# Yifei-Y/Openset-RCNN

Hardware: AMD Instinct MI355X
Metric: images/sec at 3x800x1333, R50-FPN, 1/2/4/8 MI355X; mAP_k vs ref (higher is better)
Workload: dtype f16; 1 GPU; VOC-COCO openset_rcnn_R50_FPN_128k.yaml, inference-only, 3x800x1333 uint8 BGR -> padded 800x1344, 1000 proposals/level (4273/img), 1000 dets/img, 50+50 final; batch_per_gpu=16, global_batch=16, parallelism=dp1 (images sharded, no collective), detections_last_step=1600, unknown_detections_last_step=800, known_detections_last_step=800, micro_batch_streams=1, hipgraph=True, ranks=1, distinct_gpus=1, passes_in_flight=4, images_in_flight=64

## Files before the change

include/osr.h:

```cpp
#ifndef OSR_H_
#define OSR_H_

#include <stdint.h>

#ifdef __cplusplus
extern "C" {
#endif

#define OSR_ABI_VERSION 1

typedef int32_t osr_status;
enum {
    OSR_OK = 0,
    OSR_ERR_INVALID_ARG = -1,
    OSR_ERR_UNSUPPORTED = -2,
    OSR_ERR_LAUNCH = -3,
    OSR_ERR_WORKSPACE = -4
};

typedef enum { OSR_F32 = 0, OSR_F16 = 1, OSR_BF16 = 2 } osr_dtype;

#define OSR_MAX_LEVELS 8

int32_t osr_abi_version(void);
const char* osr_last_error(void);

int32_t osr_stem_padded_width(int32_t wp);
osr_status osr_preprocess(const void* src, int32_t src_is_u8, int32_t n, int32_t h, int32_t w, int32_t hp, int32_t wp,
                          const float mean[3], const float std[3], void* dst, int32_t dst_dtype, void* stream);

typedef struct osr_conv_params {
    int32_t n, hi, wi, cin;
    int32_t ho, wo, cout;
    int32_t kh, kw, stride_h, stride_w, pad_h, pad_w;
    int64_t in_stride_n, in_stride_h, in_stride_w;
    int64_t out_stride_n, out_stride_h, out_stride_w;
    int64_t res_stride_n, res_stride_h, res_stride_w;
    int32_t relu;
    int32_t res_mode;
    int32_t pad_mode;
    int32_t in_dtype;
    int32_t out_dtype;
    int32_t concurrency;
    void* workspace;
    int64_t workspace_bytes;
    const int32_t* row_seg_counts;
    int32_t row_seg_rows;
} osr_conv_params;

int64_t osr_conv2d_fwd_workspace_bytes(const osr_conv_params* p);
int32_t osr_conv2d_fwd_describe(const osr_conv_params* p, int32_t has_workspace, char* buf, int32_t buf_bytes);

osr_status osr_conv2d_fwd(const osr_conv_params* p, const void* in, const void* weight, const float* bias,
                          const void* residual, void* out, void* stream);
osr_status osr_conv2d_fwd_masked(const osr_conv_params* p, const void* in, const void* weight, const float* bias,
                                 const void* residual, const void* mask, void* out, void* stream);

osr_status osr_conv2d_chain_fwd(const osr_conv_params* p, const void* in, const void* weight, const float* bias, const void* w3,
                                const float* bias3, int32_t cout3, const void* residual, void* out, void* stream);
osr_status osr_conv2d_chain_fwd_ex(const osr_conv_params* p, const void* in, const void* weight, const float* bias, const void* w3,
                                   const float* bias3, int32_t cout3, const void* residual, void* out, void* mid_out,
                                   void* stream);

typedef struct osr_bottleneck_params {
    int32_t n, h, w;
    int32_t cin, cmid, cout;
    int32_t dtype;
    int32_t has_proj;
} osr_bottleneck_params;
osr_status osr_bottleneck_fwd(const osr_bottleneck_params* p, const void* in, const void* w1, const float* b1,
                              const void* w2, const float* b2, const void* w3, const float* b3, const void* wsc,
                              const float* bsc, void* out, void* stream);

int64_t osr_resize_tmp_bytes(int32_t rows, int32_t nw);
osr_status osr_resize_bilinear_u8(const uint8_t* in, int32_t h, int32_t w, int64_t in_row_stride, const int32_t* xbounds,
                                  const int32_t* xcoef, int32_t kx, const int32_t* ybounds, const int32_t* ycoef,
                                  int32_t ky, int32_t y_first, int32_t y_rows, int32_t nh, int32_t nw, uint8_t* tmp,
                                  int64_t tmp_bytes, uint8_t* out, void* stream);

osr_status osr_resize_bilinear_u8_planar(const uint8_t* in, int32_t planes, int32_t h, int32_t w, const int32_t* xbounds,
                                         const int32_t* xcoef, int32_t kx, const int32_t* ybounds, const int32_t* ycoef,
                                         int32_t ky, int32_t y_first, int32_t y_rows, int32_t nh, int32_t nw, int32_t mirror,
                                         uint8_t* tmp, int64_t tmp_bytes, uint8_t* out, void* stream);

osr_status osr_stem_maxpool_fwd(const void* xpad, int32_t n, int32_t hp, int32_t wp, const void* w_view, int32_t w_rows, const float* bias,
                                void* out, int32_t dtype, void* stream);
osr_status osr_stem_maxpool_fwd_raw(const void* src, int32_t src_is_u8, int32_t n, int32_t h, int32_t w, int32_t hp, int32_t wp,
                                    const float mean[3], const float std[3], const void* w_view, int32_t w_rows, const float* bias,
                                    void* out, int32_t dtype, void* stream);
osr_status osr_stem_pool_bwd(const void* s, const void* dpool, int32_t n, int32_t hs, int32_t ws, int32_t c, void* ds, int32_t dtype,
                             void* stream);
int64_t osr_stem_wgrad_workspace_bytes(int32_t n, int32_t hp, int32_t wp);
osr_status osr_stem_wgrad(const void* xpad, const void* ds, int32_t n, int32_t hp, int32_t wp, float* dw, int32_t accumulate, void* workspace,
                          int64_t workspace_bytes, int32_t dtype, void* stream);
osr_status osr_maxpool3x3s2(const void* in, int32_t n, int32_t hi, int32_t wi, int32_t c, void* out, int32_t dtype,
                            void* stream);
osr_status osr_subsample2(const void* in, int32_t n, int32_t hi, int32_t wi, int32_t c, void* out, int32_t dtype,
                          void* stream);

osr_status osr_gemm_f32(const float* a, int64_t lda, const float* w, const float* bias, float* out, int64_t ldo,
                        int32_t m, int32_t n, int32_t k, int32_t relu, void* stream);
int64_t osr_gemm_f32_tn_workspace_bytes(int32_t m, int32_t n, int32_t k);
osr_status osr_gemm_f32_tn(const float* a, int64_t lda, const float* b, int64_t ldb, float* out, int64_t ldo, int32_t m,
                           int32_t n, int32_t k, void* workspace, int64_t workspace_bytes, void* stream);

typedef struct osr_linear_split_params {
    int32_t m, n, k;
    int32_t relu;
    int64_t ldx, ldo;
    const int32_t* row_seg_counts;
    int32_t row_seg_rows;
    int32_t reserved;
} osr_linear_split_params;
osr_status osr_split_rows_bf16(const float* w, int32_t rows, int32_t cols, void* hi, void* lo, void* stream);
osr_status osr_linear_split_fwd(const osr_linear_split_params* p, const float* x, const void* w_hi, const void* w_lo,
                                const float* bias, float* out, void* stream);

osr_status osr_split_rows_bf16_t(const float* w, int32_t rows, int32_t cols, void* hi, void* lo, void* stream);
osr_status osr_linear_split_dgrad(const float* dy, int64_t lddy, const void* wt_hi, const void* wt_lo, const float* mask,
                                  int64_t ldmask, float* dx, int64_t lddx, int32_t m, int32_t n, int32_t k,
                                  const int32_t* row_seg_counts, int32_t row_seg_rows, void* stream);
int64_t osr_linear_split_wgrad_workspace_bytes(int32_t m, int32_t n, int32_t k);
osr_status osr_linear_split_wgrad(const float* dy, int64_t lddy, const float* x, int64_t ldx, float* dw, int64_t lddw,
                                  int32_t m, int32_t n, int32_t k, const int32_t* row_seg_counts, int32_t row_seg_rows,
                                  void* workspace, int64_t workspace_bytes, void* stream);

osr_status osr_conv2d_split_fwd(const osr_conv_params* p, const float* in, const void* w_hi, const void* w_lo,
                                const float* bias, const float* residual, float* out, void* stream);

osr_status osr_cfrpn_head_tail(const void* t, int32_t t_dtype, int64_t rows, int32_t c, const float* w_delta,
                               const float* b_delta, const float* w_ctr, const float* b_ctr, float* deltas,
                               float* ctr, void* stream);

osr_status osr_cfrpn_head_fwd(const osr_conv_params* p, const void* in, const void* weight, const float* bias,
                              const float* w_tail, const float* b_tail, float* deltas, float* ctr, void* stream);
osr_status osr_conv2d_fwd_pair(const osr_conv_params* p, const void* in, const void* w_a, const float* bias_a, int32_t cout_a,
                               int32_t relu_a, void* out_a, const void* w_b, const float* bias_b, int32_t cout_b, int32_t relu_b,
                               void* out_b, void* stream);

typedef struct osr_conv_level {
    const void* in;
    void* out;
    float* deltas;
    float* ctr;
    const void* weight;
    const float* bias;
    int32_t n, hi, wi;
    int32_t reserved;
} osr_conv_level;
#define OSR_MAX_CONV_LEVELS 6
osr_status osr_conv2d_fwd_levels(const osr_conv_params* p, int32_t nlevels, const osr_conv_level* levels, const void* weight,
                                 const float* bias, void* stream);
osr_status osr_cfrpn_head_fwd_levels(const osr_conv_params* p, int32_t nlevels, const osr_conv_level* levels, const void* weight,
                                     const float* bias, const float* w_tail, const float* b_tail, void* stream);
osr_status osr_cfrpn_head_fwd_ex(const osr_conv_params* p, const void* in, const void* weight, const float* bias,
                                 const float* w_tail, const float* b_tail, float* deltas, float* ctr, void* hidden_out,
                                 void* stream);

typedef struct osr_rpn_levels {
    int32_t num_levels;
    int32_t num_anchors;
    int32_t h[OSR_MAX_LEVELS];
    int32_t w[OSR_MAX_LEVELS];
    int32_t stride[OSR_MAX_LEVELS];
    int64_t offset[OSR_MAX_LEVELS];
} osr_rpn_levels;

int32_t osr_rpn_select_capacity(const osr_rpn_levels* lv, int32_t pre_nms_topk);
int64_t osr_rpn_select_workspace_bytes(const osr_rpn_levels* lv, int32_t n, int32_t pre_nms_topk);
osr_status osr_rpn_select(const osr_rpn_levels* lv, const float* cell_anchors , const float* ctr,
                          const float* deltas, int32_t n, const int32_t* image_hw , int32_t pre_nms_topk,
                          float min_box_size, float* boxes, float* scores, int32_t* src_index, int32_t* batch_idx,
                          int32_t* counts, int32_t* status_flags, void* workspace, int64_t workspace_bytes,
                          void* stream);

osr_status osr_rpn_select_ex(const osr_rpn_levels* lv, const float* cell_anchors, const float* ctr, const float* deltas,
                             int32_t n, const int32_t* image_hw, int32_t pre_nms_topk, float min_box_size,
                             int32_t decode_mode, const float reg_weights[4], float* boxes, float* scores,
                             int32_t* src_index, int32_t* batch_idx, int32_t* level_out, int32_t* counts,
                             int32_t* status_flags, void* workspace, int64_t workspace_bytes, void* stream);

typedef struct osr_pyramid {
    int32_t num_levels;
    int32_t c;
    int32_t h[OSR_MAX_LEVELS];
    int32_t w[OSR_MAX_LEVELS];
    float scale[OSR_MAX_LEVELS];
    const void* data[OSR_MAX_LEVELS];
} osr_pyramid;

#define OSR_ROI_MAX_POOLED_FWD 14
osr_status osr_roi_align_fwd(const osr_pyramid* feats, int32_t feat_dtype, int32_t n, const float* boxes,
                             const int32_t* batch_idx, int64_t m, int32_t pooled, int32_t canonical_level,
                             int32_t canonical_size, int32_t min_level, void* out, int32_t out_dtype, void* stream);

osr_status osr_roi_align_fwd_ordered(const osr_pyramid* feats, int32_t feat_dtype, int32_t n, const float* boxes,
                                     const int32_t* batch_idx, int64_t m, int32_t pooled, int32_t canonical_level,
                                     int32_t canonical_size, int32_t min_level, const int32_t* order,
                                     const int32_t* order_nvalid, void* out, int32_t out_dtype, void* stream);
#define OSR_ROI_NO_PADDING_FILL 1
osr_status osr_roi_align_fwd_ordered_ex(const osr_pyramid* feats, int32_t feat_dtype, int32_t n, const float* boxes,
                                        const int32_t* batch_idx, int64_t m, int32_t pooled, int32_t canonical_level,
                                        int32_t canonical_size, int32_t min_level, const int32_t* order,
                                        const int32_t* order_nvalid, int32_t flags, void* out, int32_t out_dtype, void* stream);
#define OSR_ROI_MAX_SAMPLING_RATIO 64
typedef struct osr_roi_options {
    int32_t aligned;
    int32_t sampling_ratio;
} osr_roi_options;
osr_status osr_roi_align_fwd_ordered_opt(const osr_pyramid* feats, int32_t feat_dtype, int32_t n, const float* boxes,
                                         const int32_t* batch_idx, int64_t m, int32_t pooled, int32_t canonical_level,
                                         int32_t canonical_size, int32_t min_level, const int32_t* order,
                                         const int32_t* order_nvalid, int32_t flags, const osr_roi_options* options, void* out,
                                         int32_t out_dtype, void* stream);
int64_t osr_roi_locality_order_workspace_bytes(int32_t n, int64_t m);
osr_status osr_roi_locality_order(const osr_pyramid* feats, int32_t n, const float* boxes, const int32_t* batch_idx, int64_t m,
                                  int32_t canonical_level, int32_t canonical_size, int32_t min_level, int32_t* order,
                                  int32_t* nvalid, void* workspace, int64_t workspace_bytes, void* stream);

osr_status osr_box_predictor_tail(const float* x, int64_t m, int32_t k, const float* w, const float* b,
                                  const float* proposals, const float* ctr, const int32_t* batch_idx,
                                  const int32_t* image_hw, const float reg_weights[4], int32_t mean_type,
                                  float score_thresh, float* pred_deltas, float* pred_iou, float* boxes,
                                  float* score, int32_t* cand, void* stream);

int64_t osr_nms_topk_workspace_bytes(int32_t num_segments, int64_t seg_stride);
osr_status osr_nms_topk(const float* boxes, const float* scores, const int32_t* cls ,
                        const int32_t* cand , int32_t num_segments, int64_t seg_stride,
                        const int32_t* seg_len, float thr, int32_t topk, int32_t* keep, int32_t* keep_count,
                        void* workspace, int64_t workspace_bytes, void* stream);

osr_status osr_gather_rows(const float* src, int64_t seg_stride, int32_t row_elems, const int32_t* keep,
                           const int32_t* keep_count, int32_t num_segments, int32_t topk, float* dst, void* stream);

osr_status osr_l2_normalize_rows(const float* x, int32_t rows, int32_t d, float* out, void* stream);

osr_status osr_pln_tail(const float* emb, int64_t rows, int32_t d, const float* protos_normed, int32_t num_known,
                        int32_t reps, float unk_thr, int64_t unknown_id, const int64_t* class_map,
                        const int32_t* rows_valid, int32_t seg_rows, int64_t* pred_class, float* min_dist,
                        void* stream);
enum { OSR_PLN_DIST_COS = 0, OSR_PLN_DIST_L1 = 1, OSR_PLN_DIST_L2 = 2 };
osr_status osr_pln_tail_ex(const float* emb, int64_t rows, int32_t d, const float* protos_normed, int32_t num_known,
                           int32_t reps, int32_t distance_type, float unk_thr, int64_t unknown_id,
                           const int64_t* class_map, const int32_t* rows_valid, int32_t seg_rows, int64_t* pred_class,
                           float* min_dist, void* stream);

osr_status osr_softmax_candidates(const float* logits, int32_t num_known, const float* det_boxes,
                                  const float* det_scores, const int64_t* pred_class, const int32_t* det_count,
                                  int32_t n, int32_t seg_rows, int64_t unknown_id, float known_thresh,
                                  float unknown_thresh, float* k_boxes, float* k_scores, int32_t* k_cls, int32_t* k_det,
                                  int32_t* k_count, float* u_boxes, float* u_scores, int32_t* u_det, int32_t* u_count,
                                  void* stream);

osr_status osr_fastrcnn_candidates(const float* logits, const float* deltas, int32_t num_classes,
                                   int32_t num_bbox_reg_classes, const float* prop_boxes, const int32_t* prop_count,
                                   int32_t n, int32_t seg_rows, const int32_t* image_hw, const float reg_weights[4],
                                   float score_thresh, float* c_boxes, float* c_scores, int32_t* c_cls, int32_t* c_row,
                                   int32_t* c_count, void* stream);

osr_status osr_assemble_detections(const float* k_boxes, const float* k_scores, const int32_t* k_cls,
                                   const int32_t* k_keep, const int32_t* k_keep_count, int64_t k_stride, int32_t k_topk,
                                   const float* u_boxes, const float* u_scores, const int32_t* u_keep,
                                   const int32_t* u_keep_count, int64_t u_stride, int32_t u_topk, int32_t n,
                                   int64_t unknown_id, const int64_t* class_map, float* out_boxes, float* out_scores,
                                   int64_t* out_classes, int32_t* out_count, void* stream);

osr_status osr_detector_postprocess(const float* boxes, const float* scores, const int64_t* classes, const int32_t* count,
                                    int32_t n, int32_t cap, const float* scale_xy, const int32_t* out_hw, float* out_boxes,
                                    float* out_scores, int64_t* out_classes, int32_t* out_count, void* stream);

osr_status osr_mask_upsample_predict(const void* x, int32_t dtype, int64_t r, int32_t s, int32_t cin, int32_t cmid,
                                     const void* w_packed, const float* bias, const float* pred_w, const float* pred_b,
                                     int32_t num_rows, const int64_t* classes, const int32_t* rows_valid, int32_t seg_rows,
                                     float* probs, void* stream);
osr_status osr_mask_upsample_predict_ex(const void* x, int32_t dtype, int64_t r, int32_t s, int32_t cin, int32_t cmid,
                                        const void* w_packed, const float* bias, const float* pred_w, const float* pred_b,
                                        int32_t num_rows, const int64_t* classes, const int32_t* rows_valid, int32_t seg_rows,
                                        float* probs, float* logits, void* stream);
osr_status osr_paste_masks(const float* probs, const float* boxes, int64_t r, int32_t m, int32_t out_h, int32_t out_w,
                           float threshold, uint8_t* out, void* stream);

int64_t osr_mask_upsample_predict_bwd_workspace_bytes(int64_t r, int32_t s, int32_t cmid);
osr_status osr_mask_upsample_predict_bwd(const void* x, int32_t dtype, int64_t r, int32_t s, int32_t cin, int32_t cmid,
                                         const void* w_packed, const void* w_packed_t, const float* bias, const float* pred_w,
                                         int32_t num_rows, const int64_t* classes, const int32_t* rows_valid, int32_t seg_rows,
                                         const float* d_logits, void* dx, int32_t dx_dtype, void* g_out, float* d_pred_w, float* d_pred_b,
                                         float* d_deconv_b, void* workspace, int64_t workspace_bytes, void* stream);
osr_status osr_mask_targets(const uint8_t* gt_masks, int32_t n, int32_t gmax, int32_t hm, int32_t wm, const int32_t* image_hw,
                            const float* boxes, const int32_t* gt_idx, const int32_t* rows_valid, int32_t seg_rows,
                            int32_t m_side, uint8_t* targets, void* stream);
osr_status osr_mask_loss_fwd(const float* logits, const uint8_t* targets, int64_t rows, int32_t m_side, int32_t num_rows,
                             const int64_t* classes, const int32_t* rows_valid, int32_t seg_rows, float loss_weight, float* out6,
                             void* workspace, int64_t workspace_bytes, void* stream);
osr_status osr_mask_loss_bwd(const float* logits, const uint8_t* targets, int64_t rows, int32_t m_side, int32_t num_rows,
                             const int64_t* classes, const int32_t* rows_valid, int32_t seg_rows, float scale, float* d_logits,
                             void* workspace, int64_t workspace_bytes, void* stream);

osr_status osr_tta_boxes_to_original(const float* boxes, const float* scores, const int64_t* classes, const int32_t* counts,
                                     const int32_t* sizes, int32_t n, int32_t topk, int32_t ha, int32_t wa, int32_t flip,
                                     int32_t slot, int32_t cap, float* c_boxes, float* c_scores, int32_t* c_cls,
                                     int32_t* c_cand, void* stream);
osr_status osr_tta_boxes_to_augmented(const float* boxes, const int32_t* counts, const int32_t* sizes, int32_t n, int32_t topk,
                                      int32_t ha, int32_t wa, int32_t flip, float* out, void* stream);
osr_status osr_tta_reduce_masks(const float* maps, const int32_t* flip, int32_t num_aug, const int32_t* counts, int32_t n,
                                int32_t topk, int32_t m, float* out, void* stream);


osr_status osr_rpn_match_anchors(const osr_rpn_levels* levels, const float* cell_anchors, int32_t n,
                                 const float* gt_boxes, const int32_t* gt_count, int32_t gmax, float reg_lo,
                                 float reg_hi, float obj_lo, float obj_hi, int32_t* matched_idx, float* matched_iou,
                                 int8_t* labels_reg, int8_t* labels_obj, void* workspace, int64_t workspace_bytes,
                                 void* stream);

osr_status osr_subsample_labels(int8_t* labels, const float* keys, int32_t n, int64_t r, int32_t num_samples,
                                float positive_fraction, int32_t* num_pos_out, int32_t* num_neg_out, void* stream);

osr_status osr_rpn_anchor_targets(const osr_rpn_levels* levels, const float* cell_anchors, int32_t n,
                                  const float* gt_boxes, const int32_t* gt_count, int32_t gmax,
                                  const int32_t* matched_idx, const int8_t* labels_obj, float* matched_boxes,
                                  float* ctr_target, void* stream);

osr_status osr_rpn_losses_fwd(const osr_rpn_levels* levels, const float* cell_anchors, int32_t n,
                              const float* pred_deltas, const float* pred_ctr, const int8_t* labels_reg,
                              const int8_t* labels_obj, const float* matched_boxes, const float* ctr_target,
                              float loc_weight, float ctr_weight, int32_t batch_size_per_image, float* out6,
                              void* workspace, int64_t workspace_bytes, void* stream);
enum { OSR_BOX_LOSS_IOU = 0, OSR_BOX_LOSS_SMOOTH_L1 = 1, OSR_BOX_LOSS_GIOU = 2, OSR_BOX_LOSS_DIOU = 3, OSR_BOX_LOSS_CIOU = 4 };
typedef struct osr_loss_options {
    int32_t box_loss_type;
    float box_smooth_l1_beta;
    float aux_smooth_l1_beta;
} osr_loss_options;
osr_status osr_rpn_losses_fwd_ex(const osr_rpn_levels* levels, const float* cell_anchors, int32_t n,
                                 const float* pred_deltas, const float* pred_ctr, const int8_t* labels_reg,
                                 const int8_t* labels_obj, const float* matched_boxes, const float* ctr_target,
                                 float loc_weight, float ctr_weight, int32_t batch_size_per_image,
                                 const osr_loss_options* options, float* out6, void* workspace, int64_t workspace_bytes,
                                 void* stream);

int64_t osr_roi_match_sample_workspace_bytes(int32_t n, int64_t pcap, int32_t gmax);
osr_status osr_roi_match_and_sample(const float* prop_boxes, const float* prop_logits, const int32_t* prop_count,
                                    int64_t pcap, const float* gt_boxes, const int64_t* gt_classes,
                                    const int32_t* gt_count, int32_t gmax, int32_t n, const float* keys,
                                    int32_t num_classes, int32_t batch_size, float positive_fraction, float iou_thr,
                                    float* out_boxes, float* out_logits, int64_t* out_classes, float* out_ious,
                                    float* out_gt_boxes, int32_t* out_src, int32_t* out_batch_idx, int32_t* out_counts,
                                    void* workspace, int64_t workspace_bytes, void* stream);
osr_status osr_roi_match_and_sample_ex(const float* prop_boxes, const float* prop_logits, const int32_t* prop_count,
                                       int64_t pcap, const float* gt_boxes, const int64_t* gt_classes,
                                       const int32_t* gt_count, int32_t gmax, int32_t n, const float* keys,
                                       int32_t num_classes, int32_t batch_size, float positive_fraction, float iou_thr,
                                       float* out_boxes, float* out_logits, int64_t* out_classes, float* out_ious,
                                       float* out_gt_boxes, int32_t* out_src, int32_t* out_batch_idx, int32_t* out_counts,
                                       int32_t* out_gt_idx, void* workspace, int64_t workspace_bytes, void* stream);

osr_status osr_roi_box_losses_fwd(const float* pred_deltas, int32_t delta_stride, const float* pred_iou,
                                  int32_t iou_stride, int32_t iou_is_logit, const float* proposal_boxes,
                                  const float* gt_boxes, const int64_t* gt_classes, const float* gt_iou, int64_t m,
                                  int32_t num_classes, const float reg_weights[4], float box_weight, float iou_weight,
                                  float* out3, void* workspace, int64_t workspace_bytes, void* stream);
osr_status osr_roi_box_losses_fwd_ex(const float* pred_deltas, int32_t delta_stride, const float* pred_iou,
                                     int32_t iou_stride, int32_t iou_is_logit, const float* proposal_boxes,
                                     const float* gt_boxes, const int64_t* gt_classes, const float* gt_iou, int64_t m,
                                     int32_t num_classes, const float reg_weights[4], float box_weight, float iou_weight,
                                     const osr_loss_options* options, float* out3, void* workspace,
                                     int64_t workspace_bytes, void* stream);

osr_status osr_pln_loss_fwd(const float* emb, int64_t m, int32_t d, const float* protos_normed, int32_t num_known,
                            const int64_t* gt_classes, const float* ious, float iou_thr, float alpha, float beta,
                            float loss_weight, float* out1, void* workspace, int64_t workspace_bytes, void* stream);
osr_status osr_pln_loss_fwd_ex(const float* emb, int64_t m, int32_t d, const float* protos_normed, int32_t num_known,
                               int32_t reps, int32_t distance_type, const int64_t* gt_classes, const float* ious,
                               float iou_thr, float alpha, float beta, float loss_weight, float* out1, void* workspace,
                               int64_t workspace_bytes, void* stream);

// ... 173 lines not shown
```

openset-rcnn_amd/csrc/osr_bottleneck.hip:

```cpp
#include "osr_common.h"

typedef float f32x4 __attribute__((ext_vector_type(4)));
typedef f16_t bnf16x8 __attribute__((ext_vector_type(8)));
typedef bf16_t bnbf16x8 __attribute__((ext_vector_type(8)));
typedef unsigned bnu32x4 __attribute__((ext_vector_type(4)));
typedef __attribute__((address_space(3))) void bn_lds_void_t;

template <class T> struct BnFrag;
template <> struct BnFrag<f16_t> {
    typedef bnf16x8 type;
    static __device__ __forceinline__ f32x4 mfma(bnf16x8 a, bnf16x8 b, f32x4 c) { return __builtin_amdgcn_mfma_f32_16x16x32_f16(a, b, c, 0, 0, 0); }
};
template <> struct BnFrag<bf16_t> {
    typedef bnbf16x8 type;
    static __device__ __forceinline__ f32x4 mfma(bnbf16x8 a, bnbf16x8 b, f32x4 c) { return __builtin_amdgcn_mfma_f32_16x16x32_bf16(a, b, c, 0, 0, 0); }
};

struct BnArgs {
    const void* x;
    void* y;
    const void *w1, *w2, *w3, *wsc;
    const float *b1, *b2, *b3, *bsc;
    int n, h, w;
    int tiles_y, tiles_x;
    unsigned x_bytes, y_bytes, w1_bytes, w2_bytes, w3_bytes, wsc_bytes;
#ifdef BN_STAMPS
    unsigned long long* dbg;
#endif
};

#ifdef BN_STAMPS
static unsigned long long* g_bn_stamps = nullptr;
extern "C" void osr_debug_set_bn_stamps(unsigned long long* p) { g_bn_stamps = p; }
#define BN_STAMP(i) if (a.dbg && tid == 0) a.dbg[(long long)blockIdx.x * 8 + (i)] = __builtin_amdgcn_s_memrealtime()
#else
#define BN_STAMP(i)
#endif

#define BN_TH 8
#define BN_TW 16
#define BN_HW 18
#define BN_NHALO 180
#define BN_MID1 0
#define BN_MID2 24576
#define BN_WBUF 40960
#define BN_BIAS 73728
#define BN_LDS (73728 + 384 * 4)
#define BN_OOB 0x80000000u

__device__ __forceinline__ int bn_nmap(int rho) {
    const int T = rho >> 4, i = rho & 15;
    return 32 * (T >> 1) + 8 * (i >> 2) + 4 * (T & 1) + (i & 3);
}

template <class TI> __device__ __forceinline__ typename BnFrag<TI>::type bn_as_frag(bnu32x4 v) {
    union { bnu32x4 u; typename BnFrag<TI>::type f; } c;
    c.u = v;
    return c.f;
}

template <class TI, int CIN, int PROJ>
__global__ __launch_bounds__(256, 2) void bottleneck64_kernel(BnArgs a) {
    typedef typename BnFrag<TI>::type frag_t;
    constexpr int NK32 = CIN / 32, NKS = CIN / 64;
    static_assert(CIN == 64 || CIN == 256, "res2 blocks only");
    static_assert(PROJ ? CIN == 64 : CIN == 256, "identity shortcut needs cin == cout");
    extern __shared__ __attribute__((aligned(1024))) unsigned char lds[];

    const int tid = threadIdx.x, lane = tid & 63;
    const int wid = __builtin_amdgcn_readfirstlane(tid >> 6);
    const int l15 = lane & 15, g = lane >> 4;
    BN_STAMP(0);

    int t;
    {
        const int nwg = gridDim.x, b = blockIdx.x, q = nwg >> 3, r = nwg & 7, xcd = b & 7, idx = b >> 3;
        t = (xcd < r ? xcd * (q + 1) : r * (q + 1) + (xcd - r) * q) + idx;
    }
    const int tx = t % a.tiles_x, ty = (t / a.tiles_x) % a.tiles_y, img = t / (a.tiles_x * a.tiles_y);
    const int y0 = ty * BN_TH, x0 = tx * BN_TW;

    const __amdgpu_buffer_rsrc_t rs_x = __builtin_amdgcn_make_buffer_rsrc(const_cast<void*>(a.x), 0, a.x_bytes, 0x00020000);
    const __amdgpu_buffer_rsrc_t rs_y = __builtin_amdgcn_make_buffer_rsrc(a.y, 0, a.y_bytes, 0x00020000);
    const __amdgpu_buffer_rsrc_t rs_w1 = __builtin_amdgcn_make_buffer_rsrc(const_cast<void*>(a.w1), 0, a.w1_bytes, 0x00020000);
    const __amdgpu_buffer_rsrc_t rs_w2 = __builtin_amdgcn_make_buffer_rsrc(const_cast<void*>(a.w2), 0, a.w2_bytes, 0x00020000);
    const __amdgpu_buffer_rsrc_t rs_w3 = __builtin_amdgcn_make_buffer_rsrc(const_cast<void*>(a.w3), 0, a.w3_bytes, 0x00020000);

    {
        const int lrow = lane >> 3, slot = lane & 7;
#pragma unroll
        for (int ks = 0; ks < NKS; ++ks)
#pragma unroll
            for (int j = 0; j < 2; ++j) {
                const int piece = wid * 2 + j;
                const int rho = piece * 8 + lrow;
                const unsigned chunk = (unsigned)(slot ^ ((rho >> 1) & 7));
                const unsigned voff = (unsigned)((bn_nmap(rho) * CIN + ks * 64 + (int)chunk * 8) * 2);
                __builtin_amdgcn_raw_ptr_buffer_load_lds(rs_w1, (bn_lds_void_t*)(lds + BN_WBUF + ks * 8192 + piece * 1024), 16, voff, 0, 0, 0);
            }
        float* s_bias = reinterpret_cast<float*>(lds + BN_BIAS);
        for (int i = tid; i < 384; i += 256) {
            float v;
            if (i < 64) v = a.b1[i];
            else if (i < 128) v = a.b2[i - 64];
            else v = a.b3[i - 128] + (PROJ ? a.bsc[i - 128] : 0.f);
            s_bias[i] = v;
        }
    }

    unsigned xoff[3];
    bool hvalid[3];
#pragma unroll
    for (int i = 0; i < 3; ++i) {
        const int hr = wid * 48 + i * 16 + l15;
        const int hy = hr / BN_HW, hx = hr - hy * BN_HW;
        const int gy = y0 - 1 + hy, gx = x0 - 1 + hx;
        hvalid[i] = hr < BN_NHALO && (unsigned)gy < (unsigned)a.h && (unsigned)gx < (unsigned)a.w;
        xoff[i] = hvalid[i] ? (unsigned)((((long long)img * a.h + gy) * a.w + gx) * CIN * 2 + g * 16) : BN_OOB;
    }
    frag_t xf[3][NK32];
#pragma unroll
    for (int k = 0; k < NK32; ++k)
#pragma unroll
        for (int i = 0; i < 3; ++i) xf[i][k] = bn_as_frag<TI>(__builtin_amdgcn_raw_buffer_load_b128(rs_x, xoff[i] + k * 64, 0, 0));

    asm volatile("s_waitcnt vmcnt(0)" ::: "memory");
    __syncthreads();
    BN_STAMP(1);

#define BN_SW(row, chunk) ((row) * 128 + ((((chunk)) ^ (((row) >> 1) & 7)) << 4))
    {
        f32x4 acc[3][4];
#pragma unroll
        for (int i = 0; i < 3; ++i)
#pragma unroll
            for (int T = 0; T < 4; ++T) acc[i][T] = f32x4{0.f, 0.f, 0.f, 0.f};
#pragma unroll
        for (int k = 0; k < NK32; ++k) {
            frag_t wf[4];
#pragma unroll
            for (int T = 0; T < 4; ++T) {
                const int rho = T * 16 + l15;
                wf[T] = *reinterpret_cast<const frag_t*>(lds + BN_WBUF + (k >> 1) * 8192 + BN_SW(rho, (k & 1) * 4 + g));
            }
#pragma unroll
            for (int i = 0; i < 3; ++i)
#pragma unroll
                for (int T = 0; T < 4; ++T) acc[i][T] = BnFrag<TI>::mfma(wf[T], xf[i][k], acc[i][T]);
        }
        const float* s_b1 = reinterpret_cast<const float*>(lds + BN_BIAS);
#pragma unroll
        for (int i = 0; i < 3; ++i) {
            const int hr = wid * 48 + i * 16 + l15;
#pragma unroll
            for (int p = 0; p < 2; ++p) {
                const float4 ba = *reinterpret_cast<const float4*>(s_b1 + 32 * p + 8 * g), bb = *reinterpret_cast<const float4*>(s_b1 + 32 * p + 8 * g + 4);
                const float bias[8] = {ba.x, ba.y, ba.z, ba.w, bb.x, bb.y, bb.z, bb.w};
                frag_t o;
#pragma unroll
                for (int e = 0; e < 8; ++e) {
                    const float v = (e < 4 ? acc[i][2 * p][e] : acc[i][2 * p + 1][e - 4]) + bias[e];
                    o[e] = (TI)(hvalid[i] ? fmaxf(v, 0.f) : 0.f);
                }
                *reinterpret_cast<frag_t*>(lds + BN_MID1 + BN_SW(hr, 4 * p + g)) = o;
            }
        }
    }
    __syncthreads();
    BN_STAMP(2);

    frag_t w3f[4][2];
    frag_t wscf[PROJ ? 4 : 1][2];
#pragma unroll
    for (int T = 0; T < 4; ++T)
#pragma unroll
        for (int k = 0; k < 2; ++k) {
            const int n = wid * 64 + bn_nmap(T * 16 + l15);
            w3f[T][k] = bn_as_frag<TI>(__builtin_amdgcn_raw_buffer_load_b128(rs_w3, (unsigned)((n * 64 + k * 32 + g * 8) * 2), 0, 0));
            if constexpr (PROJ) {
                const __amdgpu_buffer_rsrc_t rs_wsc = __builtin_amdgcn_make_buffer_rsrc(const_cast<void*>(a.wsc), 0, a.wsc_bytes, 0x00020000);
                wscf[T][k] = bn_as_frag<TI>(__builtin_amdgcn_raw_buffer_load_b128(rs_wsc, (unsigned)((n * CIN + k * 32 + g * 8) * 2), 0, 0));
            }
        }

#define BN_STAGE_TAP(tap_)                                                                                                          \
    {                                                                                                                               \
        const int lrow_ = lane >> 3, slot_ = lane & 7;                                                                              \
        _Pragma("unroll") for (int j_ = 0; j_ < 2; ++j_) {                                                                          \
            const int piece_ = wid * 2 + j_;                                                                                        \
            const int rho_ = piece_ * 8 + lrow_;                                                                                    \
            const unsigned chunk_ = (unsigned)(slot_ ^ ((rho_ >> 1) & 7));                                                          \
            const unsigned voff_ = (unsigned)(((bn_nmap(rho_) * 9 + (tap_)) * 64 + (int)chunk_ * 8) * 2);                            \
            __builtin_amdgcn_raw_ptr_buffer_load_lds(rs_w2, (bn_lds_void_t*)(lds + BN_WBUF + ((tap_) & 3) * 8192 + piece_ * 1024), 16, voff_, 0, 0, 0); \
        }                                                                                                                           \
    }
    BN_STAGE_TAP(0);
    BN_STAGE_TAP(1);
    BN_STAGE_TAP(2);
    {
        f32x4 acc[2][4];
#pragma unroll
        for (int j = 0; j < 2; ++j)
#pragma unroll
            for (int T = 0; T < 4; ++T) acc[j][T] = f32x4{0.f, 0.f, 0.f, 0.f};
#pragma unroll
        for (int tap = 0; tap < 9; ++tap) {
            if (tap <= 6) asm volatile("s_waitcnt vmcnt(4) lgkmcnt(0)\n\ts_barrier" ::: "memory");
            else if (tap == 7) asm volatile("s_waitcnt vmcnt(2) lgkmcnt(0)\n\ts_barrier" ::: "memory");
            else asm volatile("s_waitcnt vmcnt(0) lgkmcnt(0)\n\ts_barrier" ::: "memory");
            if (tap + 3 < 9) BN_STAGE_TAP(tap + 3);
            const int ky = tap / 3, kx = tap - ky * 3;
            const unsigned char* wb = lds + BN_WBUF + (tap & 3) * 8192;
            frag_t wf[4][2];
#pragma unroll
            for (int T = 0; T < 4; ++T)
#pragma unroll
                for (int k = 0; k < 2; ++k) wf[T][k] = *reinterpret_cast<const frag_t*>(wb + BN_SW(T * 16 + l15, k * 4 + g));
#pragma unroll
            for (int j = 0; j < 2; ++j) {
                const int hr = (wid * 2 + j + ky) * BN_HW + kx + l15;
#pragma unroll
                for (int k = 0; k < 2; ++k) {
                    const frag_t af = *reinterpret_cast<const frag_t*>(lds + BN_MID1 + BN_SW(hr, k * 4 + g));
#pragma unroll
                    for (int T = 0; T < 4; ++T) acc[j][T] = BnFrag<TI>::mfma(wf[T][k], af, acc[j][T]);
                }
            }
        }
        const float* s_b2 = reinterpret_cast<const float*>(lds + BN_BIAS) + 64;
#pragma unroll
        for (int j = 0; j < 2; ++j) {
            const int row = (wid * 2 + j) * 16 + l15;
#pragma unroll
            for (int p = 0; p < 2; ++p) {
                const float4 ba = *reinterpret_cast<const float4*>(s_b2 + 32 * p + 8 * g), bb = *reinterpret_cast<const float4*>(s_b2 + 32 * p + 8 * g + 4);
                const float bias[8] = {ba.x, ba.y, ba.z, ba.w, bb.x, bb.y, bb.z, bb.w};
                frag_t o;
#pragma unroll
                for (int e = 0; e < 8; ++e) o[e] = (TI)fmaxf((e < 4 ? acc[j][2 * p][e] : acc[j][2 * p + 1][e - 4]) + bias[e], 0.f);
                *reinterpret_cast<frag_t*>(lds + BN_MID2 + BN_SW(row, 4 * p + g)) = o;
            }
        }
    }
    __syncthreads();
    BN_STAMP(3);

    const float* s_b3 = reinterpret_cast<const float*>(lds + BN_BIAS) + 128 + wid * 64;
    float bias3[2][8];
#pragma unroll
    for (int p = 0; p < 2; ++p) {
        const float4 ba = *reinterpret_cast<const float4*>(s_b3 + 32 * p + 8 * g), bb = *reinterpret_cast<const float4*>(s_b3 + 32 * p + 8 * g + 4);
        bias3[p][0] = ba.x; bias3[p][1] = ba.y; bias3[p][2] = ba.z; bias3[p][3] = ba.w;
        bias3[p][4] = bb.x; bias3[p][5] = bb.y; bias3[p][6] = bb.z; bias3[p][7] = bb.w;
    }
    frag_t aux[2][2][2];
    unsigned ooff[2][2];
#define BN_FETCH(buf, gi_)                                                                                                          \
    {                                                                                                                               \
        _Pragma("unroll") for (int j_ = 0; j_ < 2; ++j_) {                                                                          \
            const int gy_ = y0 + 2 * (gi_) + j_, gx_ = x0 + l15;                                                                    \
            const bool ok_ = gy_ < a.h && gx_ < a.w;                                                                                \
            const long long pix_ = ((long long)img * a.h + gy_) * a.w + gx_;                                                        \
            ooff[buf][j_] = ok_ ? (unsigned)(pix_ * 256 * 2) : BN_OOB;                                                              \
            _Pragma("unroll") for (int q_ = 0; q_ < 2; ++q_) {                                                                      \
                const unsigned off_ = !ok_ ? BN_OOB : PROJ ? (unsigned)(pix_ * CIN * 2 + (q_ * 32 + g * 8) * 2)                      \
                                                           : (unsigned)(pix_ * 256 * 2 + (wid * 64 + 32 * q_ + 8 * g) * 2);          \
                aux[buf][j_][q_] = bn_as_frag<TI>(__builtin_amdgcn_raw_buffer_load_b128(rs_x, off_, 0, 0));                          \
            }                                                                                                                       \
        }                                                                                                                           \
    }
    BN_FETCH(0, 0);
#pragma unroll
    for (int gi = 0; gi < 4; ++gi) {
        const int cur = gi & 1;
        if (gi + 1 < 4) { BN_FETCH((gi + 1) & 1, gi + 1); }
        f32x4 acc[2][4];
#pragma unroll
        for (int j = 0; j < 2; ++j)
#pragma unroll
            for (int T = 0; T < 4; ++T) acc[j][T] = f32x4{0.f, 0.f, 0.f, 0.f};
#pragma unroll
        for (int j = 0; j < 2; ++j) {
            const int row = (2 * gi + j) * 16 + l15;
#pragma unroll
            for (int k = 0; k < 2; ++k) {
                const frag_t af = *reinterpret_cast<const frag_t*>(lds + BN_MID2 + BN_SW(row, k * 4 + g));
#pragma unroll
                for (int T = 0; T < 4; ++T) acc[j][T] = BnFrag<TI>::mfma(w3f[T][k], af, acc[j][T]);
            }
            if constexpr (PROJ) {
#pragma unroll
                for (int k = 0; k < 2; ++k)
#pragma unroll
                    for (int T = 0; T < 4; ++T) acc[j][T] = BnFrag<TI>::mfma(wscf[T][k], aux[cur][j][k], acc[j][T]);
            }
        }
#pragma unroll
        for (int j = 0; j < 2; ++j)
#pragma unroll
            for (int p = 0; p < 2; ++p) {
                frag_t o;
#pragma unroll
                for (int e = 0; e < 8; ++e) {
                    float v = (e < 4 ? acc[j][2 * p][e] : acc[j][2 * p + 1][e - 4]) + bias3[p][e];
                    if constexpr (!PROJ) v += (float)aux[cur][j][p][e];
                    o[e] = (TI)fmaxf(v, 0.f);
                }
                union { frag_t f; bnu32x4 u; } cv;
                cv.f = o;
                __builtin_amdgcn_raw_buffer_store_b128(cv.u, rs_y, ooff[cur][j] == BN_OOB ? BN_OOB : ooff[cur][j] + (unsigned)((wid * 64 + 32 * p + 8 * g) * 2), 0, 0);
            }
    }
    BN_STAMP(4);
#ifdef BN_STAMPS
    asm volatile("s_waitcnt vmcnt(0)" ::: "memory");
    BN_STAMP(5);
#endif
}

template <class TI>
static osr_status bottleneck_launch(const osr_bottleneck_params* p, BnArgs& a, hipStream_t st) {
    const unsigned grid = (unsigned)(a.n * a.tiles_y * a.tiles_x);
    if (p->has_proj) {
        static osr_dev_mask m{0};
        osr_once_per_device(m, [] { (void)hipFuncSetAttribute(reinterpret_cast<const void*>(bottleneck64_kernel<TI, 64, 1>), hipFuncAttributeMaxDynamicSharedMemorySize, BN_LDS); });
        hipLaunchKernelGGL((bottleneck64_kernel<TI, 64, 1>), dim3(grid), dim3(256), BN_LDS, st, a);
    } else {
        static osr_dev_mask m{0};
        osr_once_per_device(m, [] { (void)hipFuncSetAttribute(reinterpret_cast<const void*>(bottleneck64_kernel<TI, 256, 0>), hipFuncAttributeMaxDynamicSharedMemorySize, BN_LDS); });
        hipLaunchKernelGGL((bottleneck64_kernel<TI, 256, 0>), dim3(grid), dim3(256), BN_LDS, st, a);
    }
    OSR_CHECK_LAUNCH("osr_bottleneck_fwd");
    return OSR_OK;
}

extern "C" osr_status osr_bottleneck_fwd(const osr_bottleneck_params* p, const void* in, const void* w1, const float* b1, const void* w2,
                                         const float* b2, const void* w3, const float* b3, const void* wsc, const float* bsc, void* out,
                                         void* stream) {
    OSR_REQUIRE(p && in && w1 && b1 && w2 && b2 && w3 && b3 && out, OSR_ERR_INVALID_ARG, "osr_bottleneck_fwd: null pointer");
    OSR_REQUIRE(p->n >= 1 && p->h >= 1 && p->w >= 1, OSR_ERR_INVALID_ARG, "osr_bottleneck_fwd: bad geometry");
    OSR_REQUIRE(p->dtype == OSR_F16 || p->dtype == OSR_BF16, OSR_ERR_UNSUPPORTED, "osr_bottleneck_fwd: dtype must be f16/bf16");
    OSR_REQUIRE(p->cmid == 64 && p->cout == 256 && ((p->has_proj && p->cin == 64) || (!p->has_proj && p->cin == 256)), OSR_ERR_UNSUPPORTED,
                "osr_bottleneck_fwd: only the res2 shapes are fused (cmid 64, cout 256; cin 64 with a projection or cin 256 without): run "
                "three osr_conv2d_fwd launches instead");
    OSR_REQUIRE(!p->has_proj || (wsc && bsc), OSR_ERR_INVALID_ARG, "osr_bottleneck_fwd: the projection shortcut needs its weight and bias");
    OSR_REQUIRE(in != out, OSR_ERR_INVALID_ARG, "osr_bottleneck_fwd: in-place is not supported (neighbouring tiles read the halo)");
    OSR_REQUIRE((((uintptr_t)in | (uintptr_t)out | (uintptr_t)w1 | (uintptr_t)w2 | (uintptr_t)w3 | (uintptr_t)wsc | (uintptr_t)b1 | (uintptr_t)b2 | (uintptr_t)b3) & 15) == 0,
                OSR_ERR_INVALID_ARG, "osr_bottleneck_fwd: pointers must be 16-byte aligned");
    const long long px = (long long)p->n * p->h * p->w;
    const long long xb = px * p->cin * 2, yb = px * p->cout * 2;
    OSR_REQUIRE(xb < (1ll << 31) - 4096 && yb < (1ll << 31) - 4096, OSR_ERR_UNSUPPORTED, "osr_bottleneck_fwd: tensor too large for 32-bit buffer offsets");
    BnArgs a;
    a.x = in; a.y = out; a.w1 = w1; a.w2 = w2; a.w3 = w3; a.wsc = wsc; a.b1 = b1; a.b2 = b2; a.b3 = b3; a.bsc = bsc;
    a.n = p->n; a.h = p->h; a.w = p->w;
    a.tiles_y = (p->h + BN_TH - 1) / BN_TH; a.tiles_x = (p->w + BN_TW - 1) / BN_TW;
#ifdef BN_STAMPS
    a.dbg = g_bn_stamps;
#endif
    a.x_bytes = (unsigned)xb; a.y_bytes = (unsigned)yb;
    a.w1_bytes = (unsigned)(64 * p->cin * 2); a.w2_bytes = 64 * 9 * 64 * 2; a.w3_bytes = 256 * 64 * 2; a.wsc_bytes = (unsigned)(256 * p->cin * 2);
    OSR_REQUIRE((long long)a.n * a.tiles_y * a.tiles_x < (1ll << 31), OSR_ERR_UNSUPPORTED, "osr_bottleneck_fwd: too many tiles");
    hipStream_t st = (hipStream_t)stream;
    return p->dtype == OSR_F16 ? bottleneck_launch<f16_t>(p, a, st) : bottleneck_launch<bf16_t>(p, a, st);
}
```

openset-rcnn_amd/host/_lib.py:

```python
from __future__ import annotations

import ctypes as C
import os

import torch

PKG_DIR = os.path.dirname(os.path.dirname(os.path.abspath(__file__)))
LIB_PATH = os.path.join(PKG_DIR, "libosr_hip.so")

OSR_MAX_LEVELS = 8
OSR_F32, OSR_F16, OSR_BF16 = 0, 1, 2
ABI_VERSION = 1


class OsrError(RuntimeError):
    pass


ERR_UNSUPPORTED = -2


class ConvParams(C.Structure):
    _fields_ = [
        ("n", C.c_int32), ("hi", C.c_int32), ("wi", C.c_int32), ("cin", C.c_int32),
        ("ho", C.c_int32), ("wo", C.c_int32), ("cout", C.c_int32),
        ("kh", C.c_int32), ("kw", C.c_int32), ("stride_h", C.c_int32), ("stride_w", C.c_int32),
        ("pad_h", C.c_int32), ("pad_w", C.c_int32),
        ("in_stride_n", C.c_int64), ("in_stride_h", C.c_int64), ("in_stride_w", C.c_int64),
        ("out_stride_n", C.c_int64), ("out_stride_h", C.c_int64), ("out_stride_w", C.c_int64),
        ("res_stride_n", C.c_int64), ("res_stride_h", C.c_int64), ("res_stride_w", C.c_int64),
        ("relu", C.c_int32), ("res_mode", C.c_int32), ("pad_mode", C.c_int32),
        ("in_dtype", C.c_int32), ("out_dtype", C.c_int32), ("concurrency", C.c_int32),
        ("workspace", C.c_void_p), ("workspace_bytes", C.c_int64),
        ("row_seg_counts", C.c_void_p), ("row_seg_rows", C.c_int32),
    ]


class ConvLevel(C.Structure):
    _fields_ = [("in_", C.c_void_p), ("out", C.c_void_p), ("deltas", C.c_void_p), ("ctr", C.c_void_p), ("weight", C.c_void_p), ("bias", C.c_void_p),
                ("n", C.c_int32), ("hi", C.c_int32), ("wi", C.c_int32), ("reserved", C.c_int32)]


MAX_CONV_LEVELS = 6


class BottleneckParams(C.Structure):
    _fields_ = [("n", C.c_int32), ("h", C.c_int32), ("w", C.c_int32), ("cin", C.c_int32), ("cmid", C.c_int32), ("cout", C.c_int32),
                ("dtype", C.c_int32), ("has_proj", C.c_int32)]


class LinearSplitParams(C.Structure):
    _fields_ = [("m", C.c_int32), ("n", C.c_int32), ("k", C.c_int32), ("relu", C.c_int32), ("ldx", C.c_int64), ("ldo", C.c_int64),
                ("row_seg_counts", C.c_void_p), ("row_seg_rows", C.c_int32), ("reserved", C.c_int32)]


class LossOptions(C.Structure):
    _fields_ = [("box_loss_type", C.c_int32), ("box_smooth_l1_beta", C.c_float), ("aux_smooth_l1_beta", C.c_float)]


BOX_LOSS_TYPES = {"iou": 0, "smooth_l1": 1, "giou": 2, "diou": 3, "ciou": 4}
PLN_DISTANCES = {"COS": 0, "L1": 1, "L2": 2}


class RpnLevels(C.Structure):
    _fields_ = [
        ("num_levels", C.c_int32), ("num_anchors", C.c_int32),
        ("h", C.c_int32 * OSR_MAX_LEVELS), ("w", C.c_int32 * OSR_MAX_LEVELS),
        ("stride", C.c_int32 * OSR_MAX_LEVELS), ("offset", C.c_int64 * OSR_MAX_LEVELS),
    ]


class SgdTensor(C.Structure):
    _fields_ = [("param", C.c_void_p), ("grad", C.c_void_p), ("momentum", C.c_void_p), ("row_scale", C.c_void_p), ("lowp", C.c_void_p),
                ("n", C.c_int64), ("row_elems", C.c_int64), ("lowp_dtype", C.c_int32), ("reserved", C.c_int32)]


class SgdSegment(C.Structure):
    _fields_ = [("param", C.c_void_p), ("grad", C.c_void_p), ("momentum", C.c_void_p), ("row_scale", C.c_void_p), ("lowp", C.c_void_p),
                ("n", C.c_int64), ("row_elems", C.c_int64), ("lowp_dtype", C.c_int32), ("chunk0", C.c_int32), ("nchunks", C.c_int32),
                ("lr_factor", C.c_float), ("weight_decay", C.c_float), ("nesterov", C.c_int32)]


OSR_CLIP_NONE, OSR_CLIP_VALUE, OSR_CLIP_NORM = 0, 1, 2


class PackTensor(C.Structure):
    _fields_ = [("src", C.c_void_p), ("dst", C.c_void_p), ("cout", C.c_int32), ("kh", C.c_int32), ("kw", C.c_int32), ("cin", C.c_int32),
                ("elem_bytes", C.c_int32), ("reserved", C.c_int32)]


class RoiOptions(C.Structure):
    _fields_ = [("aligned", C.c_int32), ("sampling_ratio", C.c_int32)]


class Pyramid(C.Structure):
    _fields_ = [
        ("num_levels", C.c_int32), ("c", C.c_int32),
        ("h", C.c_int32 * OSR_MAX_LEVELS), ("w", C.c_int32 * OSR_MAX_LEVELS),
        ("scale", C.c_float * OSR_MAX_LEVELS), ("data", C.c_void_p * OSR_MAX_LEVELS),
    ]


P, I32, I64, F32 = C.c_void_p, C.c_int32, C.c_int64, C.c_float
F32x3, F32x4 = C.c_float * 3, C.c_float * 4

PROTOTYPES = {
    "osr_abi_version": (I32, []),
    "osr_last_error": (C.c_char_p, []),
    "osr_stem_padded_width": (I32, [I32]),
    "osr_preprocess": (I32, [P, I32, I32, I32, I32, I32, I32, C.POINTER(C.c_float), C.POINTER(C.c_float), P, I32, P]),
    "osr_conv2d_fwd": (I32, [C.POINTER(ConvParams), P, P, P, P, P, P]),
    "osr_conv2d_fwd_workspace_bytes": (I64, [C.POINTER(ConvParams)]),
    "osr_conv2d_fwd_describe": (I32, [C.POINTER(ConvParams), I32, P, I32]),
    "osr_conv2d_fwd_masked": (I32, [C.POINTER(ConvParams), P, P, P, P, P, P, P]),
    "osr_conv2d_chain_fwd": (I32, [C.POINTER(ConvParams), P, P, P, P, P, I32, P, P, P]),
    "osr_conv2d_chain_fwd_ex": (I32, [C.POINTER(ConvParams), P, P, P, P, P, I32, P, P, P, P]),
    "osr_bottleneck_fwd": (I32, [C.POINTER(BottleneckParams), P, P, P, P, P, P, P, P, P, P, P]),
    "osr_resize_tmp_bytes": (I64, [I32, I32]),
    "osr_resize_bilinear_u8": (I32, [P, I32, I32, I64, P, P, I32, P, P, I32, I32, I32, I32, I32, P, I64, P, P]),
    "osr_resize_bilinear_u8_planar": (I32, [P, I32, I32, I32, P, P, I32, P, P, I32, I32, I32, I32, I32, I32, P, I64, P, P]),
    "osr_stem_maxpool_fwd": (I32, [P, I32, I32, I32, P, I32, P, P, I32, P]),
    "osr_stem_maxpool_fwd_raw": (I32, [P, I32, I32, I32, I32, I32, I32, C.POINTER(C.c_float), C.POINTER(C.c_float), P, I32, P, P, I32, P]),
    "osr_maxpool3x3s2": (I32, [P, I32, I32, I32, I32, P, I32, P]),
    "osr_stem_pool_bwd": (I32, [P, P, I32, I32, I32, I32, P, I32, P]),
    "osr_stem_wgrad_workspace_bytes": (I64, [I32, I32, I32]),
    "osr_stem_wgrad": (I32, [P, P, I32, I32, I32, P, I32, P, I64, I32, P]),
    "osr_subsample2": (I32, [P, I32, I32, I32, I32, P, I32, P]),
    "osr_gemm_f32": (I32, [P, I64, P, P, P, I64, I32, I32, I32, I32, P]),
    "osr_gemm_f32_tn_workspace_bytes": (I64, [I32, I32, I32]),
    "osr_gemm_f32_tn": (I32, [P, I64, P, I64, P, I64, I32, I32, I32, P, I64, P]),
    "osr_split_rows_bf16": (I32, [P, I32, I32, P, P, P]),
    "osr_linear_split_fwd": (I32, [C.POINTER(LinearSplitParams), P, P, P, P, P, P]),
    "osr_conv2d_split_fwd": (I32, [C.POINTER(ConvParams), P, P, P, P, P, P, P]),
    "osr_split_rows_bf16_t": (I32, [P, I32, I32, P, P, P]),
    "osr_linear_split_dgrad": (I32, [P, I64, P, P, P, I64, P, I64, I32, I32, I32, P, I32, P]),
    "osr_linear_split_wgrad_workspace_bytes": (I64, [I32, I32, I32]),
    "osr_linear_split_wgrad": (I32, [P, I64, P, I64, P, I64, I32, I32, I32, P, I32, P, I64, P]),
    "osr_cfrpn_head_tail": (I32, [P, I32, I64, I32, P, P, P, P, P, P, P]),
    "osr_cfrpn_head_fwd": (I32, [C.POINTER(ConvParams), P, P, P, P, P, P, P, P]),
    "osr_cfrpn_head_fwd_ex": (I32, [C.POINTER(ConvParams), P, P, P, P, P, P, P, P, P]),
    "osr_conv2d_fwd_pair": (I32, [C.POINTER(ConvParams), P, P, P, I32, I32, P, P, P, I32, I32, P, P]),
    "osr_conv2d_fwd_levels": (I32, [C.POINTER(ConvParams), I32, C.POINTER(ConvLevel), P, P, P]),
    "osr_cfrpn_head_fwd_levels": (I32, [C.POINTER(ConvParams), I32, C.POINTER(ConvLevel), P, P, P, P, P]),
    "osr_rpn_select_capacity": (I32, [C.POINTER(RpnLevels), I32]),
    "osr_rpn_select_workspace_bytes": (I64, [C.POINTER(RpnLevels), I32, I32]),
    "osr_rpn_select": (I32, [C.POINTER(RpnLevels), P, P, P, I32, P, I32, F32, P, P, P, P, P, P, P, I64, P]),
    "osr_rpn_select_ex": (I32, [C.POINTER(RpnLevels), P, P, P, I32, P, I32, F32, I32, P, P, P, P, P, P, P, P, P, I64, P]),
    "osr_fastrcnn_candidates": (I32, [P, P, I32, I32, P, P, I32, I32, P, P, F32, P, P, P, P, P, P]),
    "osr_roi_align_fwd": (I32, [C.POINTER(Pyramid), I32, I32, P, P, I64, I32, I32, I32, I32, P, I32, P]),
    "osr_roi_align_fwd_ordered": (I32, [C.POINTER(Pyramid), I32, I32, P, P, I64, I32, I32, I32, I32, P, P, P, I32, P]),
    "osr_roi_align_fwd_ordered_ex": (I32, [C.POINTER(Pyramid), I32, I32, P, P, I64, I32, I32, I32, I32, P, P, I32, P, I32, P]),
    "osr_roi_align_fwd_ordered_opt": (I32, [C.POINTER(Pyramid), I32, I32, P, P, I64, I32, I32, I32, I32, P, P, I32, C.POINTER(RoiOptions), P, I32, P]),
    "osr_roi_locality_order_workspace_bytes": (I64, [I32, I64]),
    "osr_roi_locality_order": (I32, [C.POINTER(Pyramid), I32, P, P, I64, I32, I32, I32, P, P, P, I64, P]),
    "osr_box_predictor_tail": (I32, [P, I64, I32, P, P, P, P, P, P, C.POINTER(C.c_float), I32, F32, P, P, P, P, P, P]),
    "osr_nms_topk_workspace_bytes": (I64, [I32, I64]),
    "osr_nms_topk": (I32, [P, P, P, P, I32, I64, P, F32, I32, P, P, P, I64, P]),
    "osr_gather_rows": (I32, [P, I64, I32, P, P, I32, I32, P, P]),
    "osr_l2_normalize_rows": (I32, [P, I32, I32, P, P]),
    "osr_pln_tail": (I32, [P, I64, I32, P, I32, I32, F32, I64, P, P, I32, P, P, P]),
    "osr_pln_tail_ex": (I32, [P, I64, I32, P, I32, I32, I32, F32, I64, P, P, I32, P, P, P]),
    "osr_softmax_candidates": (I32, [P, I32, P, P, P, P, I32, I32, I64, F32, F32, P, P, P, P, P, P, P, P, P, P]),
    "osr_assemble_detections": (I32, [P, P, P, P, P, I64, I32, P, P, P, P, I64, I32, I32, I64, P, P, P, P, P, P]),
    "osr_detector_postprocess": (I32, [P, P, P, P, I32, I32, P, P, P, P, P, P, P]),
    "osr_mask_upsample_predict": (I32, [P, I32, I64, I32, I32, I32, P, P, P, P, I32, P, P, I32, P, P]),
    "osr_paste_masks": (I32, [P, P, I64, I32, I32, I32, F32, P, P]),
    "osr_mask_targets": (I32, [P, I32, I32, I32, I32, P, P, P, P, I32, I32, P, P]),
    "osr_mask_loss_fwd": (I32, [P, P, I64, I32, I32, P, P, I32, F32, P, P, I64, P]),
    "osr_mask_loss_bwd": (I32, [P, P, I64, I32, I32, P, P, I32, F32, P, P, I64, P]),
    "osr_mask_upsample_predict_ex": (I32, [P, I32, I64, I32, I32, I32, P, P, P, P, I32, P, P, I32, P, P, P]),
    "osr_mask_upsample_predict_bwd_workspace_bytes": (I64, [I64, I32, I32]),
    "osr_mask_upsample_predict_bwd": (I32, [P, I32, I64, I32, I32, I32, P, P, P, P, I32, P, P, I32, P, P, I32, P, P, P, P, P, I64, P]),
    "osr_tta_boxes_to_original": (I32, [P, P, P, P, P, I32, I32, I32, I32, I32, I32, I32, P, P, P, P, P]),
    "osr_tta_boxes_to_augmented": (I32, [P, P, P, I32, I32, I32, I32, I32, P, P]),
    "osr_tta_reduce_masks": (I32, [P, P, I32, P, I32, I32, I32, P, P]),
    "osr_rpn_match_anchors": (I32, [P, P, I32, P, P, I32, F32, F32, F32, F32, P, P, P, P, P, I64, P]),
    "osr_subsample_labels": (I32, [P, P, I32, I64, I32, F32, P, P, P]),
    "osr_rpn_anchor_targets": (I32, [P, P, I32, P, P, I32, P, P, P, P, P]),
    "osr_rpn_losses_fwd": (I32, [P, P, I32, P, P, P, P, P, P, F32, F32, I32, P, P, I64, P]),
    "osr_rpn_losses_fwd_ex": (I32, [P, P, I32, P, P, P, P, P, P, F32, F32, I32, P, P, P, I64, P]),
    "osr_roi_match_sample_workspace_bytes": (I64, [I32, I64, I32]),
    "osr_roi_match_and_sample": (I32, [P, P, P, I64, P, P, P, I32, I32, P, I32, I32, F32, F32, P, P, P, P, P, P, P, P, P, I64, P]),
    "osr_roi_match_and_sample_ex": (I32, [P, P, P, I64, P, P, P, I32, I32, P, I32, I32, F32, F32, P, P, P, P, P, P, P, P, P, P, I64, P]),
    "osr_roi_box_losses_fwd": (I32, [P, I32, P, I32, I32, P, P, P, P, I64, I32, P, F32, F32, P, P, I64, P]),
    "osr_roi_box_losses_fwd_ex": (I32, [P, I32, P, I32, I32, P, P, P, P, I64, I32, P, F32, F32, P, P, P, I64, P]),
    "osr_pln_loss_fwd": (I32, [P, I64, I32, P, I32, P, P, F32, F32, F32, F32, P, P, I64, P]),
    "osr_pln_loss_fwd_ex": (I32, [P, I64, I32, P, I32, I32, I32, P, P, F32, F32, F32, F32, P, P, I64, P]),
    "osr_softmax_ce_loss_fwd": (I32, [P, I64, I32, P, I32, F32, P, P, I64, P]),
    "osr_conv2d_wgrad_workspace_bytes": (I64, [P]),
    "osr_conv2d_wgrad": (I32, [P, P, P, P, I32, P, I64, P]),
    "osr_conv2d_dgrad_s2": (I32, [P, P, P, P, P, P, P]),
    "osr_bias_grad": (I32, [P, I32, I64, I32, P, I32, P, I64, P]),
    "osr_rpn_losses_bwd": (I32, [P, P, I32, P, P, P, P, P, P, F32, F32, I32, F32, P, P]),
    "osr_rpn_losses_bwd_ex": (I32, [P, P, I32, P, P, P, P, P, P, F32, F32, I32, F32, P, P, P]),
    "osr_cfrpn_tail_bwd_workspace_bytes": (I64, []),
    "osr_cfrpn_tail_bwd": (I32, [P, I32, I64, P, P, P, P, P, I32, P, I64, P]),
    "osr_rpn_sparse_rows_workspace_bytes": (I64, []),
    "osr_rpn_sparse_rows": (I32, [P, I64, I32, P, P, P, P, I64, P]),
    "osr_rpn_gather_cols": (I32, [P, P, I32, I32, P, I32, P, P, P, P]),
    "osr_rpn_scatter_cols_add": (I32, [P, I32, P, P, P, I32, P]),
    "osr_roi_box_losses_bwd": (I32, [P, P, P, P, P, I64, I32, P, F32, F32, F32, P, P, I64, P]),
    "osr_roi_box_losses_bwd_ex": (I32, [P, P, P, P, P, I64, I32, P, F32, F32, F32, P, P, P, I64, P]),
    "osr_softmax_ce_loss_bwd": (I32, [P, I64, I32, P, I32, F32, F32, P, P, I64, P]),
    "osr_std_rpn_losses_fwd": (I32, [P, P, I32, P, P, P, P, P, F32, F32, F32, I32, P, P, I64, P]),
    "osr_std_rpn_losses_bwd": (I32, [P, P, I32, P, P, P, P, P, F32, F32, F32, I32, F32, P, P]),
    "osr_fastrcnn_losses_fwd": (I32, [P, P, I32, I32, P, P, P, I64, I32, P, F32, F32, F32, P, P, I64, P]),
    "osr_fastrcnn_losses_bwd": (I32, [P, P, I32, I32, P, P, P, I64, I32, P, F32, F32, F32, F32, P, P, P, I64, P]),
    "osr_std_rpn_tail_bwd_workspace_bytes": (I64, []),
    "osr_std_rpn_tail_bwd": (I32, [P, I64, P, I32, P, P, I32, P, P, P, I64, P]),
    "osr_rpn_sparse_rows_ex": (I32, [P, I64, I32, I32, P, P, P, P, I64, P]),
    "osr_rpn_gather_cols_ex": (I32, [P, P, I32, I32, P, I32, P, I32, P, P, P]),
    "osr_pln_loss_bwd_workspace_bytes": (I64, [I64]),
    "osr_pln_loss_bwd": (I32, [P, I64, I32, P, I32, P, P, F32, F32, F32, F32, F32, P, P, I32, P, I64, P]),
    "osr_pln_loss_bwd_ex": (I32, [P, I64, I32, P, I32, I32, I32, P, P, F32, F32, F32, F32, F32, P, P, I32, P, I64, P]),
    "osr_roi_align_bwd": (I32, [P, I32, P, P, I64, I32, I32, I32, I32, P, I32, P]),
    "osr_roi_align_bwd_dense": (I32, [P, I32, P, P, I64, I32, I32, I32, I32, I32, P, I32, I32, P]),
    "osr_roi_align_bwd_opt": (I32, [P, I32, P, P, I64, I32, I32, I32, I32, P, I32, C.POINTER(RoiOptions), P]),
    "osr_roi_align_bwd_dense_opt": (I32, [P, I32, P, P, I64, I32, I32, I32, I32, I32, P, I32, I32, C.POINTER(RoiOptions), P]),
    "osr_relu_mask": (I32, [P, I32, P, I32, I64, P]),
    "osr_add_cast": (I32, [P, P, P, I32, I64, P]),
    "osr_pool_bwd": (I32, [P, I32, I32, P, P, I32, I32, I32, I32, I32, I32, P]),
    "osr_sgd_step": (I32, [P, P, P, I64, F32, F32, F32, F32, P, I64, P, I32, P, P]),
    "osr_check_finite": (I32, [P, I64, P, P]),
    "osr_pack_dgrad_weight": (I32, [P, P, I32, I32, I32, I32, I32, P]),
    "osr_sgd_step_multi": (I32, [P, P, I32, I32, F32, F32, F32, F32, P, P]),
    "osr_pack_dgrad_weight_multi": (I32, [P, P, I32, P]),
    "osr_grad_norm_partials": (I32, [P, P, I32, I32, F32, F32, P, P, P]),
    "osr_sgd_step_multi_ex": (I32, [P, P, I32, I32, F32, F32, F32, I32, F32, F32, P, P, P]),
}

_lib = None


def load() -> C.CDLL:
    global _lib
    if _lib is not None:
        return _lib
    if not os.path.exists(LIB_PATH):
        raise OsrError(f"{LIB_PATH} is missing: build it with `python -c 'import __graft_entry__ as g; g.build()'` "
                       "(hipcc --offload-arch=gfx950). There is no fallback path.")
    lib = C.CDLL(LIB_PATH)
    for name, (res, args) in PROTOTYPES.items():
        fn = getattr(lib, name)
        fn.restype = res
        fn.argtypes = args
    ver = lib.osr_abi_version()
    if ver != ABI_VERSION:
        raise OsrError(f"libosr_hip.so ABI version {ver} != binding version {ABI_VERSION}")
    _lib = lib
    return lib


def check(status: int, name: str) -> None:
    if status != 0:
        msg = load().osr_last_error()
        raise OsrError(f"{name} failed (status {status}): {msg.decode() if msg else ''}")
```

openset-rcnn_amd/host/ops.py:

```python
from __future__ import annotations

import ctypes as C
from typing import Dict, List, Optional, Sequence, Tuple

import torch

from . import _lib
from ._lib import ConvParams, OsrError, Pyramid, RpnLevels, check

_DT = {torch.float32: _lib.OSR_F32, torch.float16: _lib.OSR_F16, torch.bfloat16: _lib.OSR_BF16}


def _p(t: Optional[torch.Tensor]):
    return None if t is None else C.c_void_p(t.data_ptr())


def _stream():
    return C.c_void_p(torch.cuda.current_stream().cuda_stream)


def _need(t: torch.Tensor, dtype=None, name="tensor"):
    if not t.is_cuda:
        raise OsrError(f"{name} must live on the GPU (got {t.device}); the HIP path has no CPU fallback")
    if dtype is not None and t.dtype != dtype:
# ... 93 lines not shown
    wo = (wi + 2 * pad - kw) // stride + 1
    out_dtype = out_dtype or x.dtype
    if out is None:
        out = torch.empty((n, ho, wo, cout), dtype=out_dtype, device=x.device)
    else:
        _need(out, out_dtype, "out")
        assert out.numel() == n * ho * wo * cout
    if FLOP_COUNT is not None:
        FLOP_COUNT["conv"] += 2.0 * n * ho * wo * cout * kh * kw * cin
    p = _conv_params(n, hi, wi, cin, ho, wo, cout, kh, kw, stride, pad, x.dtype, out_dtype, relu, res_mode)
    if row_seg is not None:
        counts, seg_rows = row_seg
        _need(counts, torch.int32, "row_seg counts")
        if seg_rows < 1 or counts.numel() * seg_rows < n * ho * wo:
            raise OsrError("row_seg does not cover the output rows")
        p.row_seg_counts, p.row_seg_rows = counts.data_ptr(), int(seg_rows)
    if res_mode:
        _set_residual(p, residual, x.dtype)
    if post_mask is not None:
        _need(post_mask, x.dtype, "post_mask")
        if tuple(post_mask.shape) != (n, ho, wo, cout):
            raise OsrError(f"post_mask shape {tuple(post_mask.shape)} != {(n, ho, wo, cout)}")
        st = lib.osr_conv2d_fwd_masked(C.byref(p), _p(x), _p(weight), _p(bias), _p(residual) if res_mode else None, _p(post_mask), _p(out),
                                       _stream())
        if st != _lib.ERR_UNSUPPORTED:
            check(st, "osr_conv2d_fwd_masked")
            return out
    ws = None
    if SPLIT_K_TAIL and post_mask is None and res_mode == 0 and stride == 1:
        wsb = int(lib.osr_conv2d_fwd_workspace_bytes(C.byref(p)))
        if wsb > 0:
            ws = torch.empty((wsb,), dtype=torch.uint8, device=x.device)
            p.workspace, p.workspace_bytes = ws.data_ptr(), wsb
    check(lib.osr_conv2d_fwd(C.byref(p), _p(x), _p(weight), _p(bias), _p(residual) if res_mode else None, _p(out), _stream()),
          "osr_conv2d_fwd")
    if post_mask is not None:
        relu_mask_(out, post_mask)
    return out


def stem_conv(xpad: torch.Tensor, w_view: torch.Tensor, bias: torch.Tensor, hp: int, wp: int, relu: bool = True) -> torch.Tensor:
    lib = _lib.load()
    _need(xpad, name="xpad"); _need(w_view, xpad.dtype, "w_view"); _need(bias, torch.float32, "bias")
    n, hd, wd, c4 = xpad.shape
    assert c4 == 4 and hd == hp + 6 and wd == stem_padded_width(wp)
    cout = w_view.shape[0]
    assert tuple(w_view.shape[1:]) in ((7, 1, 32), (8, 1, 32))
    kh = w_view.shape[1]
    ho, wo = hp // 2, wp // 2
    out = torch.empty((n, ho, wo, cout), dtype=xpad.dtype, device=xpad.device)
    if FLOP_COUNT is not None:
        FLOP_COUNT["conv"] += 2.0 * n * ho * wo * cout * 147
    p = _stem_params(n, hd, wd, ho, wo, cout, kh, relu, xpad.dtype)
    check(lib.osr_conv2d_fwd(C.byref(p), _p(xpad), _p(w_view), _p(bias), None, _p(out), _stream()), "osr_conv2d_fwd(stem)")
    return out


def stem_maxpool(xpad: torch.Tensor, w_view: torch.Tensor, bias: torch.Tensor, hp: int, wp: int) -> torch.Tensor:
    lib = _lib.load()
    _need(xpad, name="xpad"); _need(w_view, xpad.dtype, "w_view"); _need(bias, torch.float32, "bias")
    n, hd, wd, c4 = xpad.shape
    assert c4 == 4 and hd == hp + 6 and wd == stem_padded_width(wp) and hp % 2 == 0 and wp % 2 == 0
    assert w_view.shape[0] == 64 and tuple(w_view.shape[2:]) == (1, 32) and w_view.shape[1] in (7, 8)
    hs, ws = hp // 2, wp // 2
    out = torch.empty((n, (hs - 1) // 2 + 1, (ws - 1) // 2 + 1, 64), dtype=xpad.dtype, device=xpad.device)
    if FLOP_COUNT is not None:
        FLOP_COUNT["conv"] += 2.0 * n * hs * ws * 64 * 147
    check(lib.osr_stem_maxpool_fwd(_p(xpad), n, hp, wp, _p(w_view), int(w_view.shape[1]), _p(bias), _p(out), _DT[xpad.dtype], _stream()), "osr_stem_maxpool_fwd")
    return out


def stem_maxpool_raw(images: torch.Tensor, hp: int, wp: int, mean, std, w_view: torch.Tensor, bias: torch.Tensor) -> torch.Tensor:
    lib = _lib.load()
    _need(images, name="images"); _need(w_view, name="w_view"); _need(bias, torch.float32, "bias")
    if images.dtype not in (torch.uint8, torch.float32) or w_view.dtype not in (torch.float16, torch.bfloat16):
        raise OsrError("stem_maxpool_raw: uint8 / float32 images, f16 / bf16 weights")
    n, c, h, w = images.shape
    assert c == 3 and hp >= h and wp >= w and hp % 2 == 0 and wp % 2 == 0
    assert w_view.shape[0] == 64 and tuple(w_view.shape[2:]) == (1, 32) and w_view.shape[1] in (7, 8)
    hs, ws = hp // 2, wp // 2
    out = torch.empty((n, (hs - 1) // 2 + 1, (ws - 1) // 2 + 1, 64), dtype=w_view.dtype, device=images.device)
    if FLOP_COUNT is not None:
        FLOP_COUNT["conv"] += 2.0 * n * hs * ws * 64 * 147
    m = (C.c_float * 3)(*[float(v) for v in mean])
    s = (C.c_float * 3)(*[float(v) for v in std])
    check(lib.osr_stem_maxpool_fwd_raw(_p(images), int(images.dtype == torch.uint8), n, h, w, hp, wp, m, s, _p(w_view), int(w_view.shape[1]), _p(bias),
                                       _p(out), _DT[w_view.dtype], _stream()), "osr_stem_maxpool_fwd_raw")
    return out


def linear(x: torch.Tensor, weight: torch.Tensor, bias: torch.Tensor, relu: bool = False,
           out_dtype: Optional[torch.dtype] = None, row_seg: Optional[Tuple[torch.Tensor, int]] = None) -> torch.Tensor:
    m, k = x.shape
    y = conv2d(x.view(1, m, 1, k), weight.view(weight.shape[0], 1, 1, k), bias, relu=relu, out_dtype=out_dtype, row_seg=row_seg)
    return y.view(m, weight.shape[0])


LINEAR_SPLIT_COUNT = None


def _split_planes(w: torch.Tensor, shape, out, name: str):
    _need(w, torch.float32, "w")
    if w.dim() != 2 or w.numel() == 0:
        raise OsrError(f"{name}: a non-empty 2-d matrix")
    if out is None:
        return torch.empty(shape, dtype=torch.bfloat16, device=w.device), torch.empty(shape, dtype=torch.bfloat16, device=w.device)
    hi, lo = out[0], out[1]
    _need(hi, torch.bfloat16, "out hi"); _need(lo, torch.bfloat16, "out lo")
    if tuple(hi.shape) != tuple(shape) or tuple(lo.shape) != tuple(shape):
        raise OsrError(f"{name}: the planes must be {tuple(shape)}")
    return hi, lo


def split_rows_bf16(w: torch.Tensor, out=None) -> Tuple[torch.Tensor, torch.Tensor]:
    hi, lo = _split_planes(w, tuple(w.shape), out, "split_rows_bf16")
    check(_lib.load().osr_split_rows_bf16(_p(w), w.shape[0], w.shape[1], _p(hi), _p(lo), _stream()), "osr_split_rows_bf16")
    return hi, lo


def split_rows_bf16_t(w: torch.Tensor, out=None) -> Tuple[torch.Tensor, torch.Tensor]:
    hi, lo = _split_planes(w, tuple(w.shape[::-1]), out, "split_rows_bf16_t")
    check(_lib.load().osr_split_rows_bf16_t(_p(w), w.shape[0], w.shape[1], _p(hi), _p(lo), _stream()), "osr_split_rows_bf16_t")
    return hi, lo


LINEAR_SPLIT_DGRAD_COUNT = None
LINEAR_SPLIT_WGRAD_COUNT = None


def _row_seg_args(row_seg, m: int):
    if row_seg is None:
        return None, 0
    counts, seg_rows = row_seg
    _need(counts, torch.int32, "row_seg counts")
    if seg_rows < 1 or counts.numel() * seg_rows < m:
        raise OsrError("row_seg does not cover the rows")
    return counts.data_ptr(), int(seg_rows)


def linear_split_dgrad(dy: torch.Tensor, wt_split, mask: Optional[torch.Tensor] = None, row_seg: Optional[Tuple[torch.Tensor, int]] = None,
                       out: Optional[torch.Tensor] = None) -> torch.Tensor:
    hi, lo = wt_split[0], wt_split[1]
    _need(dy, torch.float32, "dy"); _need(hi, torch.bfloat16, "wt_split hi"); _need(lo, torch.bfloat16, "wt_split lo")
    if dy.dim() != 2 or hi.dim() != 2 or hi.shape != lo.shape or hi.shape[1] != dy.shape[1] or dy.shape[0] < 1:
        raise OsrError(f"linear_split_dgrad: dy {tuple(dy.shape)}, transposed weight planes {tuple(hi.shape)} / {tuple(lo.shape)}")
    (m, n), k = dy.shape, hi.shape[0]
    if mask is not None:
        _need(mask, torch.float32, "mask")
        if tuple(mask.shape) != (m, k):
            raise OsrError(f"linear_split_dgrad: mask {tuple(mask.shape)} for dx {(m, k)}")
    if out is None:
        out = torch.empty((m, k), dtype=torch.float32, device=dy.device)
    else:
        _need(out, torch.float32, "out")
        assert tuple(out.shape) == (m, k)
    seg_p, seg_rows = _row_seg_args(row_seg, m)
    check(_lib.load().osr_linear_split_dgrad(_p(dy), n, _p(hi), _p(lo), _p(mask), k, _p(out), k, m, n, k, seg_p, seg_rows, _stream()),
          "osr_linear_split_dgrad")
    if LINEAR_SPLIT_DGRAD_COUNT is not None:
        LINEAR_SPLIT_DGRAD_COUNT["launches"] += 1
        LINEAR_SPLIT_DGRAD_COUNT["flops"] += 2.0 * m * k * n
    return out


def linear_split_wgrad(x: torch.Tensor, dy: torch.Tensor, dw: Optional[torch.Tensor] = None,
                       row_seg: Optional[Tuple[torch.Tensor, int]] = None) -> torch.Tensor:
    lib = _lib.load()
    _need(x, torch.float32, "x"); _need(dy, torch.float32, "dy")
    if x.dim() != 2 or dy.dim() != 2 or x.shape[0] != dy.shape[0] or x.shape[0] < 1:
        raise OsrError(f"linear_split_wgrad: x {tuple(x.shape)}, dy {tuple(dy.shape)}")
    (m, k), n = x.shape, dy.shape[1]
    if dw is None:
        dw = torch.empty((n, k), dtype=torch.float32, device=x.device)
    else:
        _need(dw, torch.float32, "dw")
        assert tuple(dw.shape) == (n, k)
    seg_p, seg_rows = _row_seg_args(row_seg, m)
    nb = int(lib.osr_linear_split_wgrad_workspace_bytes(m, n, k))
    ws = torch.empty((nb,), dtype=torch.uint8, device=x.device) if nb else None
    check(lib.osr_linear_split_wgrad(_p(dy), n, _p(x), k, _p(dw), k, m, n, k, seg_p, seg_rows, _p(ws), nb, _stream()), "osr_linear_split_wgrad")
    if LINEAR_SPLIT_WGRAD_COUNT is not None:
        LINEAR_SPLIT_WGRAD_COUNT["launches"] += 1
        LINEAR_SPLIT_WGRAD_COUNT["flops"] += 2.0 * m * k * n
    return dw


def linear_split(x: torch.Tensor, w_split, bias: torch.Tensor, relu: bool = False, row_seg: Optional[Tuple[torch.Tensor, int]] = None,
                 x_exp: Optional[torch.Tensor] = None, out: Optional[torch.Tensor] = None) -> torch.Tensor:
    if x_exp is not None:
        raise OsrError("linear_split: the bf16 split carries no row exponents (x_exp must be None)")
    hi, lo = w_split[0], w_split[1]
    _need(x, torch.float32, "x"); _need(hi, torch.bfloat16, "w_split hi"); _need(lo, torch.bfloat16, "w_split lo"); _need(bias, torch.float32, "bias")
    if x.dim() != 2 or hi.dim() != 2 or hi.shape != lo.shape or hi.shape[1] != x.shape[1] or bias.numel() != hi.shape[0] or x.shape[0] < 1:
        raise OsrError(f"linear_split: x {tuple(x.shape)}, weight planes {tuple(hi.shape)} / {tuple(lo.shape)}, bias {tuple(bias.shape)}")
    (m, k), n = x.shape, hi.shape[0]
    if out is None:
        out = torch.empty((m, n), dtype=torch.float32, device=x.device)
    else:
        _need(out, torch.float32, "out")
        assert tuple(out.shape) == (m, n)
    p = _lib.LinearSplitParams()
    p.m, p.n, p.k, p.relu, p.ldx, p.ldo = m, n, k, int(relu), k, n
    if row_seg is not None:
        counts, seg_rows = row_seg
        _need(counts, torch.int32, "row_seg counts")
        if seg_rows < 1 or counts.numel() * seg_rows < m:
            raise OsrError("row_seg does not cover the output rows")
        p.row_seg_counts, p.row_seg_rows = counts.data_ptr(), int(seg_rows)
    check(_lib.load().osr_linear_split_fwd(C.byref(p), _p(x), _p(hi), _p(lo), _p(bias), _p(out), _stream()), "osr_linear_split_fwd")
    if LINEAR_SPLIT_COUNT is not None:
        LINEAR_SPLIT_COUNT["launches"] += 1
        LINEAR_SPLIT_COUNT["flops"] += 2.0 * m * k * n
    return out


CONV_SPLIT_COUNT = None


def _conv_split_planes(w_split, name: str):
    hi, lo = w_split[0], w_split[1]
    _need(hi, torch.bfloat16, name + " hi"); _need(lo, torch.bfloat16, name + " lo")
    if hi.dim() != 4 or hi.shape != lo.shape:
        raise OsrError(f"{name}: two (cout,kh,kw,cin) bf16 planes, got {tuple(hi.shape)} / {tuple(lo.shape)}")
    return hi, lo


def conv2d_split(x: torch.Tensor, w_split, bias: torch.Tensor, stride: int = 1, pad: int = 0, relu: bool = False,
                 residual: Optional[torch.Tensor] = None, res_mode: int = 0, out: Optional[torch.Tensor] = None) -> torch.Tensor:
    lib = _lib.load()
    _need(x, torch.float32, "x"); _need(bias, torch.float32, "bias")
    hi, lo = _conv_split_planes(w_split, "w_split")
    if x.dim() != 4:
        raise OsrError(f"conv2d_split: x must be (n,h,w,cin), got {tuple(x.shape)}")
    n, hi_, wi, cin = x.shape
    cout, kh, kw, cin2 = hi.shape
    if cin2 != cin:
        raise OsrError(f"weight cin {cin2} != input cin {cin}")
    ho = (hi_ + 2 * pad - kh) // stride + 1
    wo = (wi + 2 * pad - kw) // stride + 1
    if out is None:
        out = torch.empty((n, ho, wo, cout), dtype=torch.float32, device=x.device)
    else:
        _need(out, torch.float32, "out")
        if tuple(out.shape) not in ((n, ho, wo, cout), (n * ho * wo, cout)):
            raise OsrError(f"conv2d_split: out {tuple(out.shape)} for a result of {(n, ho, wo, cout)} (or its {(n * ho * wo, cout)} rows)")
    p = _conv_params(n, hi_, wi, cin, ho, wo, cout, kh, kw, stride, pad, torch.float32, torch.float32, relu, res_mode)
    if res_mode:
        _set_residual(p, residual, torch.float32)
    check(lib.osr_conv2d_split_fwd(C.byref(p), _p(x), _p(hi), _p(lo), _p(bias), _p(residual) if res_mode else None, _p(out), _stream()),
          "osr_conv2d_split_fwd")
    if CONV_SPLIT_COUNT is not None:
        CONV_SPLIT_COUNT["launches"] += 1
        CONV_SPLIT_COUNT["flops"] += 2.0 * n * ho * wo * cout * kh * kw * cin
    return out


def stem_conv_split(xpad: torch.Tensor, w_split, bias: torch.Tensor, hp: int, wp: int, relu: bool = True) -> torch.Tensor:
    lib = _lib.load()
    _need(xpad, torch.float32, "xpad"); _need(bias, torch.float32, "bias")
    hi, lo = _conv_split_planes(w_split, "w_split")
    n, hd, wd, c4 = xpad.shape
    assert c4 == 4 and hd == hp + 6 and wd == stem_padded_width(wp)
    cout = hi.shape[0]
    assert tuple(hi.shape[1:]) == (8, 1, 32)
    ho, wo = hp // 2, wp // 2
    out = torch.empty((n, ho, wo, cout), dtype=torch.float32, device=xpad.device)
    p = _stem_params(n, hd, wd, ho, wo, cout, 8, relu, torch.float32)
    check(lib.osr_conv2d_split_fwd(C.byref(p), _p(xpad), _p(hi), _p(lo), _p(bias), None, _p(out), _stream()), "osr_conv2d_split_fwd(stem)")
    if CONV_SPLIT_COUNT is not None:
        CONV_SPLIT_COUNT["launches"] += 1
        CONV_SPLIT_COUNT["flops"] += 2.0 * n * ho * wo * cout * 147
    return out


def conv2d_chain(x: torch.Tensor, weight: torch.Tensor, bias: torch.Tensor, w3: torch.Tensor, b3: torch.Tensor, residual: torch.Tensor,
                 stride: int = 1, pad: int = 0, keep_mid: bool = False):
    lib = _lib.load()
    _need(x, name="x")
    if x.dtype not in (torch.float16, torch.bfloat16):
        return None
    _need(weight, x.dtype, "weight"); _need(w3, x.dtype, "w3"); _need(residual, x.dtype, "residual")
    _need(bias, torch.float32, "bias"); _need(b3, torch.float32, "b3")
    n, hi, wi, cin = x.shape
    cmid, kh, kw, cin2 = weight.shape
    cout3 = w3.shape[0]
    if cin2 != cin or tuple(w3.shape) != (cout3, 1, 1, cmid) or bias.numel() != cmid or b3.numel() != cout3:
        raise OsrError("conv2d_chain: weight shapes do not form conv -> 1x1 conv")
    ho = (hi + 2 * pad - kh) // stride + 1
    wo = (wi + 2 * pad - kw) // stride + 1
    if tuple(residual.shape) != (n, ho, wo, cout3):
        raise OsrError(f"conv2d_chain: residual shape {tuple(residual.shape)} != {(n, ho, wo, cout3)}")
    p = _conv_params(n, hi, wi, cin, ho, wo, cmid, kh, kw, stride, pad, x.dtype, x.dtype, relu=True)
    out = torch.empty((n, ho, wo, cout3), dtype=x.dtype, device=x.device)
    mid = torch.empty((n, ho, wo, cmid), dtype=x.dtype, device=x.device) if keep_mid else None
    st = lib.osr_conv2d_chain_fwd_ex(C.byref(p), _p(x), _p(weight), _p(bias), _p(w3), _p(b3), cout3, _p(residual), _p(out), _p(mid), _stream())
    if st == _lib.ERR_UNSUPPORTED:
        return None
    check(st, "osr_conv2d_chain_fwd")
    if FLOP_COUNT is not None:
        FLOP_COUNT["conv"] += 2.0 * n * ho * wo * (cmid * kh * kw * cin + cout3 * cmid)
    return (out, mid) if keep_mid else out


def bottleneck(x: torch.Tensor, w1, b1, w2, b2, w3, b3, wsc=None, bsc=None) -> Optional[torch.Tensor]:
    lib = _lib.load()
    _need(x, name="x")
    if x.dtype not in (torch.float16, torch.bfloat16):
        return None
    n, h, w, cin = x.shape
    cmid, cout = w1.shape[0], w3.shape[0]
    for t, nm in ((w1, "w1"), (w2, "w2"), (w3, "w3")):
        _need(t, x.dtype, nm)
    for t, nm in ((b1, "b1"), (b2, "b2"), (b3, "b3")):
        _need(t, torch.float32, nm)
    if tuple(w1.shape) != (cmid, 1, 1, cin) or tuple(w2.shape) != (cmid, 3, 3, cmid) or tuple(w3.shape) != (cout, 1, 1, cmid):
        raise OsrError("bottleneck: weight shapes do not form a 1x1 -> 3x3 -> 1x1 block")
    p = _lib.BottleneckParams()
    p.n, p.h, p.w, p.cin, p.cmid, p.cout = n, h, w, cin, cmid, cout
    p.dtype, p.has_proj = _DT[x.dtype], int(wsc is not None)
    if wsc is not None:
        _need(wsc, x.dtype, "wsc"); _need(bsc, torch.float32, "bsc")
        if tuple(wsc.shape) != (cout, 1, 1, cin):
            raise OsrError("bottleneck: projection weight shape")
    out = torch.empty((n, h, w, cout), dtype=x.dtype, device=x.device)
    st = lib.osr_bottleneck_fwd(C.byref(p), _p(x), _p(w1), _p(b1), _p(w2), _p(b2), _p(w3), _p(b3), _p(wsc), _p(bsc), _p(out), _stream())
    if st == _lib.ERR_UNSUPPORTED:
        return None
    check(st, "osr_bottleneck_fwd")
    if FLOP_COUNT is not None:
        FLOP_COUNT["conv"] += 2.0 * n * h * w * (cin * cmid + 9 * cmid * cmid + cmid * cout + (cin * cout if wsc is not None else 0))
    return out


def resize_bilinear_u8(img: torch.Tensor, xbounds, xcoef, kx: int, ybounds, ycoef, ky: int, y_first: int, y_rows: int, nh: int, nw: int,
                       out: Optional[torch.Tensor] = None) -> torch.Tensor:
    lib = _lib.load()
    _need(img, torch.uint8, "img")
    for t, nm in ((xbounds, "xbounds"), (xcoef, "xcoef"), (ybounds, "ybounds"), (ycoef, "ycoef")):
        _need(t, torch.int32, nm)
    h, w, c = img.shape
    if c != 3 or xbounds.shape[0] != nw or ybounds.shape[0] != nh or xcoef.shape[1] != kx or ycoef.shape[1] != ky:
        raise OsrError("resize_bilinear_u8: table shapes do not match the sizes")
    tmp_bytes = int(lib.osr_resize_tmp_bytes(y_rows, nw))
    tmp = torch.empty((tmp_bytes,), dtype=torch.uint8, device=img.device)
    if out is None:
        out = torch.empty((3, nh, nw), dtype=torch.uint8, device=img.device)
    else:
        _need(out, torch.uint8, "out")
        if tuple(out.shape) != (3, nh, nw):
            raise OsrError("resize_bilinear_u8: out must be (3, nh, nw)")
    check(lib.osr_resize_bilinear_u8(_p(img), h, w, w * 3, _p(xbounds), _p(xcoef), kx, _p(ybounds), _p(ycoef), ky, y_first, y_rows, nh, nw, _p(tmp),
                                     tmp_bytes, _p(out), _stream()), "osr_resize_bilinear_u8")
    return out


def resize_bilinear_u8_planar(img: torch.Tensor, xbounds, xcoef, kx: int, ybounds, ycoef, ky: int, y_first: int, y_rows: int, nh: int, nw: int,
                              mirror: bool = False, out: Optional[torch.Tensor] = None) -> torch.Tensor:
    lib = _lib.load()
    _need(img, torch.uint8, "img")
    for t, nm in ((xbounds, "xbounds"), (xcoef, "xcoef"), (ybounds, "ybounds"), (ycoef, "ycoef")):
        _need(t, torch.int32, nm)
    if img.dim() not in (3, 4):
        raise OsrError("resize_bilinear_u8_planar: img must be (planes, h, w) or (n, planes, h, w)")
    h, w = int(img.shape[-2]), int(img.shape[-1])
    planes = img.numel() // max(h * w, 1)
    if tuple(xbounds.shape) != (nw, 2) or tuple(ybounds.shape) != (nh, 2) or tuple(xcoef.shape) != (nw, kx) or tuple(ycoef.shape) != (nh, ky):
        raise OsrError("resize_bilinear_u8_planar: table shapes do not match the sizes")
    tmp_bytes = planes * y_rows * nw
    tmp = torch.empty((tmp_bytes,), dtype=torch.uint8, device=img.device)
    shape = tuple(img.shape[:-2]) + (nh, nw)
    if out is None:
        out = torch.empty(shape, dtype=torch.uint8, device=img.device)
    else:
        _need(out, torch.uint8, "out")
        if tuple(out.shape) != shape:
            raise OsrError(f"resize_bilinear_u8_planar: out must be {shape}")
    check(lib.osr_resize_bilinear_u8_planar(_p(img), planes, h, w, _p(xbounds), _p(xcoef), kx, _p(ybounds), _p(ycoef), ky, y_first, y_rows, nh, nw,
                                            int(bool(mirror)), _p(tmp), tmp_bytes, _p(out), _stream()), "osr_resize_bilinear_u8_planar")
    return out


def maxpool3x3s2(x: torch.Tensor) -> torch.Tensor:
    lib = _lib.load()
    _need(x, name="x")
    n, h, w, c = x.shape
    out = torch.empty((n, (h - 1) // 2 + 1, (w - 1) // 2 + 1, c), dtype=x.dtype, device=x.device)
    check(lib.osr_maxpool3x3s2(_p(x), n, h, w, c, _p(out), _DT[x.dtype], _stream()), "osr_maxpool3x3s2")
    return out


def stem_pool_bwd(s: torch.Tensor, dpool: torch.Tensor) -> torch.Tensor:
    lib = _lib.load()
    _need(s, name="s"); _need(dpool, s.dtype, "dpool")
    n, hs, ws, c = s.shape
    if tuple(dpool.shape) != (n, (hs - 1) // 2 + 1, (ws - 1) // 2 + 1, c):
        raise OsrError(f"dpool shape {tuple(dpool.shape)} does not match the stem output {tuple(s.shape)}")
    ds = torch.empty_like(s)
    check(lib.osr_stem_pool_bwd(_p(s), _p(dpool), n, hs, ws, c, _p(ds), _DT[s.dtype], _stream()), "osr_stem_pool_bwd")
    return ds


def stem_wgrad(xpad: torch.Tensor, ds: torch.Tensor, hp: int, wp: int, dw: Optional[torch.Tensor] = None, accumulate: bool = False) -> torch.Tensor:
    lib = _lib.load()
    _need(xpad, name="xpad"); _need(ds, xpad.dtype, "ds")
    n = xpad.shape[0]
    if tuple(xpad.shape) != (n, hp + 6, stem_padded_width(wp), 4) or tuple(ds.shape) != (n, hp // 2, wp // 2, 64):
        raise OsrError(f"stem_wgrad: xpad {tuple(xpad.shape)} / ds {tuple(ds.shape)} do not match hp={hp}, wp={wp}")
    if dw is None:
        dw = torch.empty((64, 8, 1, 32), dtype=torch.float32, device=xpad.device)
        accumulate = False
    else:
        _need(dw, torch.float32, "dw")
        if tuple(dw.shape) != (64, 8, 1, 32):
            raise OsrError(f"stem_wgrad: dw must be (64, 8, 1, 32), got {tuple(dw.shape)}")
    wsb = int(lib.osr_stem_wgrad_workspace_bytes(n, hp, wp))
    if wsb < 0:
        check(wsb, "osr_stem_wgrad_workspace_bytes")
    ws = torch.empty((wsb,), dtype=torch.uint8, device=xpad.device)
    if FLOP_COUNT is not None:
        FLOP_COUNT["wgrad"] += 2.0 * n * (hp // 2) * (wp // 2) * 64 * 147
    check(lib.osr_stem_wgrad(_p(xpad), _p(ds), n, hp, wp, _p(dw), int(accumulate), _p(ws), wsb, _DT[xpad.dtype], _stream()), "osr_stem_wgrad")
    return dw


def subsample2(x: torch.Tensor) -> torch.Tensor:
    lib = _lib.load()
    _need(x, name="x")
    n, h, w, c = x.shape
    out = torch.empty((n, (h - 1) // 2 + 1, (w - 1) // 2 + 1, c), dtype=x.dtype, device=x.device)
    check(lib.osr_subsample2(_p(x), n, h, w, c, _p(out), _DT[x.dtype], _stream()), "osr_subsample2")
    return out


def gemm_f32(a: torch.Tensor, w: torch.Tensor, bias: Optional[torch.Tensor], relu: bool = False) -> torch.Tensor:
    lib = _lib.load()
    _need(a, torch.float32, "a"); _need(w, torch.float32, "w")
    if bias is not None:
        _need(bias, torch.float32, "bias")
    m, k = a.shape
    n = w.shape[0]
    assert w.shape[1] == k
    out = torch.empty((m, n), dtype=torch.float32, device=a.device)
    check(lib.osr_gemm_f32(_p(a), k, _p(w), _p(bias), _p(out), n, m, n, k, int(relu), _stream()), "osr_gemm_f32")
    return out


def gemm_f32_tn(a: torch.Tensor, b: torch.Tensor, out: Optional[torch.Tensor] = None) -> torch.Tensor:
    lib = _lib.load()
    _need(a, torch.float32, "a"); _need(b, torch.float32, "b")
    k, m = a.shape
    assert b.shape[0] == k
    n = b.shape[1]
    if out is None:
        out = torch.empty((m, n), dtype=torch.float32, device=a.device)
    else:
        _need(out, torch.float32, "out")
        assert tuple(out.shape) == (m, n)
    nb = int(lib.osr_gemm_f32_tn_workspace_bytes(m, n, k))
    ws = torch.empty((nb,), dtype=torch.uint8, device=a.device) if nb else None
    check(lib.osr_gemm_f32_tn(_p(a), m, _p(b), n, _p(out), n, m, n, k, _p(ws), nb, _stream()), "osr_gemm_f32_tn")
    return out


def cfrpn_head_tail(t: torch.Tensor, w_delta, b_delta, w_ctr, b_ctr) -> Tuple[torch.Tensor, torch.Tensor]:
    lib = _lib.load()
    _need(t, name="t")
    rows, c = t.shape
    for x in (w_delta, b_delta, w_ctr, b_ctr):
        _need(x, torch.float32, "head weight")
    deltas = torch.empty((rows, 4), dtype=torch.float32, device=t.device)
    ctr = torch.empty((rows,), dtype=torch.float32, device=t.device)
    check(lib.osr_cfrpn_head_tail(_p(t), _DT[t.dtype], rows, c, _p(w_delta), _p(b_delta), _p(w_ctr), _p(b_ctr), _p(deltas), _p(ctr),
                                  _stream()), "osr_cfrpn_head_tail")
    return deltas, ctr


def cfrpn_head_fused(x: torch.Tensor, weight: torch.Tensor, bias: torch.Tensor, w_tail: torch.Tensor, b_tail: torch.Tensor,
                     deltas_out: Optional[torch.Tensor] = None, ctr_out: Optional[torch.Tensor] = None, hidden_out: Optional[torch.Tensor] = None):
    lib = _lib.load()
    _need(x, name="x"); _need(weight, x.dtype, "weight"); _need(bias, torch.float32, "bias")
    _need(w_tail, torch.float32, "w_tail"); _need(b_tail, torch.float32, "b_tail")
    n, hi, wi, cin = x.shape
    cout, kh, kw, _ = weight.shape
    pad = kh // 2
    rows = n * hi * wi
    if FLOP_COUNT is not None:
        FLOP_COUNT["conv"] += 2.0 * rows * cout * (kh * kw * cin + 5)
    deltas = deltas_out if deltas_out is not None else torch.empty((rows, 4), dtype=torch.float32, device=x.device)
    ctr = ctr_out if ctr_out is not None else torch.empty((rows,), dtype=torch.float32, device=x.device)
    _need(deltas, torch.float32, "deltas"); _need(ctr, torch.float32, "ctr")
    assert deltas.numel() == rows * 4 and ctr.numel() == rows
    p = _conv_params(n, hi, wi, cin, hi, wi, cout, kh, kw, 1, pad, x.dtype, x.dtype, relu=True)
    if hidden_out is not None:
        _need(hidden_out, x.dtype, "hidden_out")
        assert hidden_out.numel() == rows * 256
    check(lib.osr_cfrpn_head_fwd_ex(C.byref(p), _p(x), _p(weight), _p(bias), _p(w_tail), _p(b_tail), _p(deltas), _p(ctr), _p(hidden_out), _stream()),
          "osr_cfrpn_head_fwd")
    return deltas, ctr


def conv2d_pair(x: torch.Tensor, w_a: torch.Tensor, b_a: torch.Tensor, relu_a: bool, w_b: torch.Tensor, b_b: torch.Tensor, relu_b: bool,
                stride: int = 1, pad: int = 0):
    lib = _lib.load()
    ca, kh, kw, cin = w_a.shape
    cb = w_b.shape[0]
    if tuple(w_b.shape[1:]) != (kh, kw, cin) or ca % 128 or cb % 128 or cin % 64 or x.dtype not in (torch.float16, torch.bfloat16):
        return None
    _need(x, name="x"); _need(w_a, x.dtype, "w_a"); _need(w_b, x.dtype, "w_b"); _need(b_a, torch.float32, "b_a"); _need(b_b, torch.float32, "b_b")
    n, hi, wi, _ = x.shape
    ho, wo = (hi + 2 * pad - kh) // stride + 1, (wi + 2 * pad - kw) // stride + 1
    out_a = torch.empty((n, ho, wo, ca), dtype=x.dtype, device=x.device)
    out_b = torch.empty((n, ho, wo, cb), dtype=x.dtype, device=x.device)
    p = _conv_params(n, hi, wi, cin, ho, wo, ca + cb, kh, kw, stride, pad, x.dtype, x.dtype)
    st = lib.osr_conv2d_fwd_pair(C.byref(p), _p(x), _p(w_a), _p(b_a), ca, int(relu_a), _p(out_a), _p(w_b), _p(b_b), cb, int(relu_b), _p(out_b), _stream())
    if st == _lib.ERR_UNSUPPORTED:
        return None
    check(st, "osr_conv2d_fwd_pair")
    if FLOP_COUNT is not None:
        FLOP_COUNT["conv"] += 2.0 * n * ho * wo * (ca + cb) * kh * kw * cin
    return out_a, out_b


def _conv_levels(xs: Sequence[torch.Tensor], outs, deltas=None, ctrs=None, weights=None, biases=None):
    assert 1 <= len(xs) <= _lib.MAX_CONV_LEVELS
    arr = (_lib.ConvLevel * len(xs))()
    for i, x in enumerate(xs):
        n, hi, wi, _ = x.shape
        arr[i].in_ = x.data_ptr()
        arr[i].out = outs[i].data_ptr() if outs is not None and outs[i] is not None else None
        arr[i].deltas = deltas[i].data_ptr() if deltas is not None else None
        arr[i].ctr = ctrs[i].data_ptr() if ctrs is not None else None
        arr[i].weight = weights[i].data_ptr() if weights is not None else None
        arr[i].bias = biases[i].data_ptr() if biases is not None else None
        arr[i].n, arr[i].hi, arr[i].wi = n, hi, wi
    return arr


def _levels_params(x0: torch.Tensor, weight: torch.Tensor, relu: bool):
    cout, kh, kw, cin = weight.shape
    assert kh == kw and kh % 2 == 1 and x0.shape[3] == cin
    p = _new_conv_params()
    p.cin, p.cout, p.kh, p.kw, p.stride_h, p.stride_w, p.pad_h, p.pad_w = cin, cout, kh, kw, 1, 1, kh // 2, kw // 2
    p.in_stride_w, p.out_stride_w = cin, cout
    p.relu, p.res_mode, p.pad_mode = 1 if relu else 0, 0, 0
    p.in_dtype = p.out_dtype = _DT[x0.dtype]
    return p


def conv2d_levels(xs: Sequence[torch.Tensor], weight, bias, relu: bool = False, outs: Optional[Sequence[torch.Tensor]] = None):
    lib = _lib.load()
    ws = list(weight) if isinstance(weight, (list, tuple)) else None
    bs = list(bias) if isinstance(bias, (list, tuple)) else None
    w0 = ws[0] if ws is not None else weight
    cout, kh, kw, cin = w0.shape
    if cout % 256 or cin % 64 or kh != kw or kh % 2 == 0 or kh * kw * cin // 64 < 2 or xs[0].dtype not in (torch.float16, torch.bfloat16) or len(xs) > _lib.MAX_CONV_LEVELS:
        return None
    assert (ws is None) == (bs is None) and (ws is None or (len(ws) == len(xs) and len(bs) == len(xs)))
    for w_, b_ in zip(ws if ws is not None else [weight], bs if bs is not None else [bias]):
        _need(w_, xs[0].dtype, "weight"); _need(b_, torch.float32, "bias")
        assert tuple(w_.shape) == (cout, kh, kw, cin) and b_.numel() == cout
    for x in xs:
        _need(x, xs[0].dtype, "x")
        assert x.shape[3] == cin
    if outs is None:
        outs = [torch.empty(tuple(x.shape[:3]) + (cout,), dtype=x.dtype, device=x.device) for x in xs]
    for x, o in zip(xs, outs):
        _need(o, x.dtype, "out")
        assert tuple(o.shape) == tuple(x.shape[:3]) + (cout,)
    if FLOP_COUNT is not None:
        FLOP_COUNT["conv"] += sum(2.0 * x.shape[0] * x.shape[1] * x.shape[2] * cout * kh * kw * cin for x in xs)
    p = _levels_params(xs[0], w0, relu)
    arr = _conv_levels(xs, outs, weights=ws, biases=bs)
    st = lib.osr_conv2d_fwd_levels(C.byref(p), len(xs), arr, None if ws is not None else _p(weight), None if bs is not None else _p(bias), _stream())
    if st == _lib.ERR_UNSUPPORTED:
        return None
    check(st, "osr_conv2d_fwd_levels")
    return list(outs)


def cfrpn_head_fused_levels(xs: Sequence[torch.Tensor], weight: torch.Tensor, bias: torch.Tensor, w_tail: torch.Tensor, b_tail: torch.Tensor,
                            deltas_outs: Sequence[torch.Tensor], ctr_outs: Sequence[torch.Tensor],
                            hidden_outs: Optional[Sequence[Optional[torch.Tensor]]] = None) -> bool:
    lib = _lib.load()
    cout, kh, kw, cin = weight.shape
    if cout != 256 or cin % 64 or kh != kw or kh % 2 == 0 or kh * kw * cin // 64 < 8 or xs[0].dtype not in (torch.float16, torch.bfloat16) or len(xs) > _lib.MAX_CONV_LEVELS:
        return False
    _need(weight, xs[0].dtype, "weight"); _need(bias, torch.float32, "bias")
    _need(w_tail, torch.float32, "w_tail"); _need(b_tail, torch.float32, "b_tail")
    for i, x in enumerate(xs):
        _need(x, xs[0].dtype, "x")
        rows = x.shape[0] * x.shape[1] * x.shape[2]
        _need(deltas_outs[i], torch.float32, "deltas"); _need(ctr_outs[i], torch.float32, "ctr")
        assert deltas_outs[i].numel() == rows * 4 and ctr_outs[i].numel() == rows and x.shape[3] == cin
        if hidden_outs is not None and hidden_outs[i] is not None:
            _need(hidden_outs[i], x.dtype, "hidden_out")
            assert hidden_outs[i].numel() == rows * 256
    if FLOP_COUNT is not None:
        FLOP_COUNT["conv"] += sum(2.0 * x.shape[0] * x.shape[1] * x.shape[2] * cout * (kh * kw * cin + 5) for x in xs)
    p = _levels_params(xs[0], weight, True)
    arr = _conv_levels(xs, hidden_outs, deltas_outs, ctr_outs)
    st = lib.osr_cfrpn_head_fwd_levels(C.byref(p), len(xs), arr, _p(weight), _p(bias), _p(w_tail), _p(b_tail), _stream())
    if st == _lib.ERR_UNSUPPORTED:
        return False
    check(st, "osr_cfrpn_head_fwd_levels")
    return True


def make_rpn_levels(shapes: Sequence[Tuple[int, int]], strides: Sequence[int], n: int, num_anchors: int = 1) -> RpnLevels:
    lv = RpnLevels()
    lv.num_levels, lv.num_anchors = len(shapes), num_anchors
    off = 0
    for i, ((h, w), s) in enumerate(zip(shapes, strides)):
        lv.h[i], lv.w[i], lv.stride[i], lv.offset[i] = h, w, s, off
        off += n * h * w * num_anchors
    return lv


def rpn_select(lv: RpnLevels, cell_anchors: torch.Tensor, ctr: torch.Tensor, deltas: torch.Tensor, n: int,
               image_hw: torch.Tensor, pre_nms_topk: int, min_box_size: float = 0.0, b2b_weights: Optional[Sequence[float]] = None):
    if b2b_weights is not None:
        return _rpn_select_ex(lv, cell_anchors, ctr, deltas, n, image_hw, pre_nms_topk, min_box_size, b2b_weights)
    lib = _lib.load()
    _need(cell_anchors, torch.float32, "cell_anchors"); _need(ctr, torch.float32, "ctr"); _need(deltas, torch.float32, "deltas")
    _need(image_hw, torch.int32, "image_hw")
    cap = lib.osr_rpn_select_capacity(C.byref(lv), pre_nms_topk)
    if cap < 0:
        check(cap, "osr_rpn_select_capacity")
    wsb = lib.osr_rpn_select_workspace_bytes(C.byref(lv), n, pre_nms_topk)
# ... 1183 lines not shown
```

Baseline: 1608 images/sec.

## Make fused res2 bottleneck kernel persistent with resident weights and prefetched halos

New measurement: 1626 images/sec, median of 6. 1.1% higher.

```diff
diff --git a/include/osr.h b/include/osr.h
--- a/include/osr.h
+++ b/include/osr.h
@@ -71,6 +71,9 @@
 osr_status osr_bottleneck_fwd(const osr_bottleneck_params* p, const void* in, const void* w1, const float* b1,
                               const void* w2, const float* b2, const void* w3, const float* b3, const void* wsc,
                               const float* bsc, void* out, void* stream);
+osr_status osr_bottleneck_fwd_ex(const osr_bottleneck_params* p, const void* in, const void* w1, const float* b1,
+                                 const void* w2, const float* b2, const void* w3, const float* b3, const void* wsc,
+                                 const float* bsc, void* out, int32_t max_workgroups, void* stream);
 
 int64_t osr_resize_tmp_bytes(int32_t rows, int32_t nw);
 osr_status osr_resize_bilinear_u8(const uint8_t* in, int32_t h, int32_t w, int64_t in_row_stride, const int32_t* xbounds,
diff --git a/openset-rcnn_amd/csrc/osr_bottleneck.hip b/openset-rcnn_amd/csrc/osr_bottleneck.hip
--- a/openset-rcnn_amd/csrc/osr_bottleneck.hip
+++ b/openset-rcnn_amd/csrc/osr_bottleneck.hip
@@ -23,6 +23,7 @@
     const float *b1, *b2, *b3, *bsc;
     int n, h, w;
     int tiles_y, tiles_x;
+    int ntiles, npairs;
     unsigned x_bytes, y_bytes, w1_bytes, w2_bytes, w3_bytes, wsc_bytes;
 #ifdef BN_STAMPS
     unsigned long long* dbg;
@@ -32,7 +33,7 @@
 #ifdef BN_STAMPS
 static unsigned long long* g_bn_stamps = nullptr;
 extern "C" void osr_debug_set_bn_stamps(unsigned long long* p) { g_bn_stamps = p; }
-#define BN_STAMP(i) if (a.dbg && tid == 0) a.dbg[(long long)blockIdx.x * 8 + (i)] = __builtin_amdgcn_s_memrealtime()
+#define BN_STAMP(i) if (a.dbg && tid == 0) a.dbg[(long long)pair * 8 + (i)] = __builtin_amdgcn_s_memrealtime()
 #else
 #define BN_STAMP(i)
 #endif
@@ -41,13 +42,13 @@
 #define BN_TW 16
 #define BN_HW 18
 #define BN_NHALO 180
-#define BN_MID1 0
-#define BN_MID2 24576
-#define BN_WBUF 40960
-#define BN_BIAS 73728
-#define BN_LDS (73728 + 384 * 4)
+#define BN_W1 0
+#define BN_W2 32768
+#define BN_BIAS 106496
+#define BN_MID 108032
+#define BN_MID_HALF 24576
+#define BN_LDS (BN_MID + 2 * BN_MID_HALF)
 #define BN_OOB 0x80000000u
-
 __device__ __forceinline__ int bn_nmap(int rho) {
     const int T = rho >> 4, i = rho & 15;
     return 32 * (T >> 1) + 8 * (i >> 2) + 4 * (T & 1) + (i & 3);
@@ -59,8 +60,25 @@
     return c.f;
 }
 
+#define BN_BARRIER() asm volatile("s_waitcnt lgkmcnt(0)\n\ts_barrier" ::: "memory")
+
+struct BnTile {
+    int y0, x0, img;
+    bool ok;
+};
+
+__device__ __forceinline__ BnTile bn_tile(const BnArgs& a, int t) {
+    BnTile r;
+    r.ok = t < a.ntiles;
+    const int tx = t % a.tiles_x, ty = (t / a.tiles_x) % a.tiles_y;
+    r.img = t / (a.tiles_x * a.tiles_y);
+    r.y0 = ty * BN_TH;
+    r.x0 = tx * BN_TW;
+    return r;
+}
+
 template <class TI, int CIN, int PROJ>
-__global__ __launch_bounds__(256, 2) void bottleneck64_kernel(BnArgs a) {
+__global__ __launch_bounds__(512) void bottleneck64_kernel(BnArgs a) {
     typedef typename BnFrag<TI>::type frag_t;
     constexpr int NK32 = CIN / 32, NKS = CIN / 64;
     static_assert(CIN == 64 || CIN == 256, "res2 blocks only");
@@ -68,199 +86,199 @@
     extern __shared__ __attribute__((aligned(1024))) unsigned char lds[];
 
     const int tid = threadIdx.x, lane = tid & 63;
-    const int wid = __builtin_amdgcn_readfirstlane(tid >> 6);
+    const int wid8 = __builtin_amdgcn_readfirstlane(tid >> 6);
+    const int half = wid8 >> 2, wid = wid8 & 3;
     const int l15 = lane & 15, g = lane >> 4;
-    BN_STAMP(0);
-
-    int t;
+    unsigned char* const mid = lds + BN_MID + half * BN_MID_HALF;
+
+    int pair, pair_end, pair_step;
     {
-        const int nwg = gridDim.x, b = blockIdx.x, q = nwg >> 3, r = nwg & 7, xcd = b & 7, idx = b >> 3;
-        t = (xcd < r ? xcd * (q + 1) : r * (q + 1) + (xcd - r) * q) + idx;
-    }
-    const int tx = t % a.tiles_x, ty = (t / a.tiles_x) % a.tiles_y, img = t / (a.tiles_x * a.tiles_y);
-    const int y0 = ty * BN_TH, x0 = tx * BN_TW;
+        const int nwg = gridDim.x, b = blockIdx.x, nx = nwg < 8 ? nwg : 8;
+        const int xcd = b & 7, idx = b >> 3;
+        const int W = (nwg - xcd + 7) >> 3;
+        const int q = a.npairs / nx, r = a.npairs - q * nx;
+        const int first = xcd * q + (xcd < r ? xcd : r), count = q + (xcd < r ? 1 : 0);
+        pair = first + idx;
+        pair_end = first + count;
+        pair_step = W;
+    }
 
     const __amdgpu_buffer_rsrc_t rs_x = __builtin_amdgcn_make_buffer_rsrc(const_cast<void*>(a.x), 0, a.x_bytes, 0x00020000);
     const __amdgpu_buffer_rsrc_t rs_y = __builtin_amdgcn_make_buffer_rsrc(a.y, 0, a.y_bytes, 0x00020000);
-    const __amdgpu_buffer_rsrc_t rs_w1 = __builtin_amdgcn_make_buffer_rsrc(const_cast<void*>(a.w1), 0, a.w1_bytes, 0x00020000);
-    const __amdgpu_buffer_rsrc_t rs_w2 = __builtin_amdgcn_make_buffer_rsrc(const_cast<void*>(a.w2), 0, a.w2_bytes, 0x00020000);
-    const __amdgpu_buffer_rsrc_t rs_w3 = __builtin_amdgcn_make_buffer_rsrc(const_cast<void*>(a.w3), 0, a.w3_bytes, 0x00020000);
 
     {
-        const int lrow = lane >> 3, slot = lane & 7;
-#pragma unroll
-        for (int ks = 0; ks < NKS; ++ks)
-#pragma unroll
-            for (int j = 0; j < 2; ++j) {
-                const int piece = wid * 2 + j;
-                const int rho = piece * 8 + lrow;
-                const unsigned chunk = (unsigned)(slot ^ ((rho >> 1) & 7));
-                const unsigned voff = (unsigned)((bn_nmap(rho) * CIN + ks * 64 + (int)chunk * 8) * 2);
-                __builtin_amdgcn_raw_ptr_buffer_load_lds(rs_w1, (bn_lds_void_t*)(lds + BN_WBUF + ks * 8192 + piece * 1024), 16, voff, 0, 0, 0);
-            }
+        const __amdgpu_buffer_rsrc_t rs_w1 = __builtin_amdgcn_make_buffer_rsrc(const_cast<void*>(a.w1), 0, a.w1_bytes, 0x00020000);
+        const __amdgpu_buffer_rsrc_t rs_w2 = __builtin_amdgcn_make_buffer_rsrc(const_cast<void*>(a.w2), 0, a.w2_bytes, 0x00020000);
+        const int rho = wid8 * 8 + (lane >> 3);
+        const unsigned chunk = (unsigned)((lane & 7) ^ ((rho >> 1) & 7));
+#pragma unroll
+        for (int ks = 0; ks < NKS; ++ks) {
+            const unsigned voff = (unsigned)((bn_nmap(rho) * CIN + ks * 64 + (int)chunk * 8) * 2);
+            __builtin_amdgcn_raw_ptr_buffer_load_lds(rs_w1, (bn_lds_void_t*)(lds + BN_W1 + ks * 8192 + wid8 * 1024), 16, voff, 0, 0, 0);
+        }
+#pragma unroll
+        for (int tap = 0; tap < 9; ++tap) {
+            const unsigned voff = (unsigned)(((bn_nmap(rho) * 9 + tap) * 64 + (int)chunk * 8) * 2);
+            __builtin_amdgcn_raw_ptr_buffer_load_lds(rs_w2, (bn_lds_void_t*)(lds + BN_W2 + tap * 8192 + wid8 * 1024), 16, voff, 0, 0, 0);
+        }
         float* s_bias = reinterpret_cast<float*>(lds + BN_BIAS);
-        for (int i = tid; i < 384; i += 256) {
+        if (tid < 384) {
             float v;
-            if (i < 64) v = a.b1[i];
-            else if (i < 128) v = a.b2[i - 64];
-            else v = a.b3[i - 128] + (PROJ ? a.bsc[i - 128] : 0.f);
-            s_bias[i] = v;
-        }
-    }
-
-    unsigned xoff[3];
+            if (tid < 64) v = a.b1[tid];
+            else if (tid < 128) v = a.b2[tid - 64];
+            else v = a.b3[tid - 128] + (PROJ ? a.bsc[tid - 128] : 0.f);
+            s_bias[tid] = v;
+        }
+    }
+    frag_t w3f[4][2];
+    frag_t wscf[PROJ ? 4 : 1][2];
+    {
+        const __amdgpu_buffer_rsrc_t rs_w3 = __builtin_amdgcn_make_buffer_rsrc(const_cast<void*>(a.w3), 0, a.w3_bytes, 0x00020000);
+#pragma unroll
+        for (int T = 0; T < 4; ++T)
+#pragma unroll
+            for (int k = 0; k < 2; ++k) {
+                const int n = wid * 64 + bn_nmap(T * 16 + l15);
+                w3f[T][k] = bn_as_frag<TI>(__builtin_amdgcn_raw_buffer_load_b128(rs_w3, (unsigned)((n * 64 + k * 32 + g * 8) * 2), 0, 0));
+                if constexpr (PROJ) {
+                    const __amdgpu_buffer_rsrc_t rs_wsc = __builtin_amdgcn_make_buffer_rsrc(const_cast<void*>(a.wsc), 0, a.wsc_bytes, 0x00020000);
+                    wscf[T][k] = bn_as_frag<TI>(__builtin_amdgcn_raw_buffer_load_b128(rs_wsc, (unsigned)((n * CIN + k * 32 + g * 8) * 2), 0, 0));
+                }
+            }
+    }
+
+    frag_t xf[3][NK32];
     bool hvalid[3];
-#pragma unroll
-    for (int i = 0; i < 3; ++i) {
-        const int hr = wid * 48 + i * 16 + l15;
-        const int hy = hr / BN_HW, hx = hr - hy * BN_HW;
-        const int gy = y0 - 1 + hy, gx = x0 - 1 + hx;
-        hvalid[i] = hr < BN_NHALO && (unsigned)gy < (unsigned)a.h && (unsigned)gx < (unsigned)a.w;
-        xoff[i] = hvalid[i] ? (unsigned)((((long long)img * a.h + gy) * a.w + gx) * CIN * 2 + g * 16) : BN_OOB;
-    }
-    frag_t xf[3][NK32];
-#pragma unroll
-    for (int k = 0; k < NK32; ++k)
-#pragma unroll
-        for (int i = 0; i < 3; ++i) xf[i][k] = bn_as_frag<TI>(__builtin_amdgcn_raw_buffer_load_b128(rs_x, xoff[i] + k * 64, 0, 0));
+    unsigned xo[3];
+#define BN_HALO_ADDR(tl)                                                                                                            \
+    {                                                                                                                               \
+        _Pragma("unroll") for (int i_ = 0; i_ < 3; ++i_) {                                                                          \
+            const int hr_ = wid * 48 + i_ * 16 + l15;                                                                               \
+            const int hy_ = hr_ / BN_HW, hx_ = hr_ - hy_ * BN_HW;                                                                   \
+            const int gy_ = (tl).y0 - 1 + hy_, gx_ = (tl).x0 - 1 + hx_;                                                             \
+            hvalid[i_] = (tl).ok && hr_ < BN_NHALO && (unsigned)gy_ < (unsigned)a.h && (unsigned)gx_ < (unsigned)a.w;               \
+            xo[i_] = hvalid[i_] ? (unsigned)((((long long)(tl).img * a.h + gy_) * a.w + gx_) * CIN * 2 + g * 16) : BN_OOB;          \
+        }                                                                                                                           \
+    }
+#define BN_HALO_LOAD(i_, k_) xf[i_][k_] = bn_as_frag<TI>(__builtin_amdgcn_raw_buffer_load_b128(rs_x, xo[i_] + (k_) * 64, 0, 0))
+    BnTile cur = bn_tile(a, 2 * pair + half), nxt;
+    if (pair >= pair_end) cur.ok = false;
+    BN_HALO_ADDR(cur);
+#pragma unroll
+    for (int i = 0; i < 3; ++i)
+#pragma unroll
+        for (int k = 0; k < NK32; ++k) BN_HALO_LOAD(i, k);
 
     asm volatile("s_waitcnt vmcnt(0)" ::: "memory");
     __syncthreads();
-    BN_STAMP(1);
 
 #define BN_SW(row, chunk) ((row) * 128 + ((((chunk)) ^ (((row) >> 1) & 7)) << 4))
-    {
-        f32x4 acc[3][4];
-#pragma unroll
-        for (int i = 0; i < 3; ++i)
-#pragma unroll
-            for (int T = 0; T < 4; ++T) acc[i][T] = f32x4{0.f, 0.f, 0.f, 0.f};
-#pragma unroll
-        for (int k = 0; k < NK32; ++k) {
-            frag_t wf[4];
-#pragma unroll
-            for (int T = 0; T < 4; ++T) {
-                const int rho = T * 16 + l15;
-                wf[T] = *reinterpret_cast<const frag_t*>(lds + BN_WBUF + (k >> 1) * 8192 + BN_SW(rho, (k & 1) * 4 + g));
-            }
+    for (; pair < pair_end; pair += pair_step) {
+        BN_STAMP(0);
+        {
+            f32x4 acc[3][4];
 #pragma unroll
             for (int i = 0; i < 3; ++i)
 #pragma unroll
-                for (int T = 0; T < 4; ++T) acc[i][T] = BnFrag<TI>::mfma(wf[T], xf[i][k], acc[i][T]);
-        }
-        const float* s_b1 = reinterpret_cast<const float*>(lds + BN_BIAS);
-#pragma unroll
-        for (int i = 0; i < 3; ++i) {
-            const int hr = wid * 48 + i * 16 + l15;
-#pragma unroll
-            for (int p = 0; p < 2; ++p) {
-                const float4 ba = *reinterpret_cast<const float4*>(s_b1 + 32 * p + 8 * g), bb = *reinterpret_cast<const float4*>(s_b1 + 32 * p + 8 * g + 4);
-                const float bias[8] = {ba.x, ba.y, ba.z, ba.w, bb.x, bb.y, bb.z, bb.w};
-                frag_t o;
-#pragma unroll
-                for (int e = 0; e < 8; ++e) {
-                    const float v = (e < 4 ? acc[i][2 * p][e] : acc[i][2 * p + 1][e - 4]) + bias[e];
-                    o[e] = (TI)(hvalid[i] ? fmaxf(v, 0.f) : 0.f);
-                }
-                *reinterpret_cast<frag_t*>(lds + BN_MID1 + BN_SW(hr, 4 * p + g)) = o;
-            }
-        }
-    }
-    __syncthreads();
-    BN_STAMP(2);
-
-    frag_t w3f[4][2];
-    frag_t wscf[PROJ ? 4 : 1][2];
-#pragma unroll
-    for (int T = 0; T < 4; ++T)
-#pragma unroll
-        for (int k = 0; k < 2; ++k) {
-            const int n = wid * 64 + bn_nmap(T * 16 + l15);
-            w3f[T][k] = bn_as_frag<TI>(__builtin_amdgcn_raw_buffer_load_b128(rs_w3, (unsigned)((n * 64 + k * 32 + g * 8) * 2), 0, 0));
-            if constexpr (PROJ) {
-                const __amdgpu_buffer_rsrc_t rs_wsc = __builtin_amdgcn_make_buffer_rsrc(const_cast<void*>(a.wsc), 0, a.wsc_bytes, 0x00020000);
-                wscf[T][k] = bn_as_frag<TI>(__builtin_amdgcn_raw_buffer_load_b128(rs_wsc, (unsigned)((n * CIN + k * 32 + g * 8) * 2), 0, 0));
-            }
-        }
-
-#define BN_STAGE_TAP(tap_)                                                                                                          \
-    {                                                                                                                               \
-        const int lrow_ = lane >> 3, slot_ = lane & 7;                                                                              \
-        _Pragma("unroll") for (int j_ = 0; j_ < 2; ++j_) {                                                                          \
-            const int piece_ = wid * 2 + j_;                                                                                        \
-            const int rho_ = piece_ * 8 + lrow_;                                                                                    \
-            const unsigned chunk_ = (unsigned)(slot_ ^ ((rho_ >> 1) & 7));                                                          \
-            const unsigned voff_ = (unsigned)(((bn_nmap(rho_) * 9 + (tap_)) * 64 + (int)chunk_ * 8) * 2);                            \
-            __builtin_amdgcn_raw_ptr_buffer_load_lds(rs_w2, (bn_lds_void_t*)(lds + BN_WBUF + ((tap_) & 3) * 8192 + piece_ * 1024), 16, voff_, 0, 0, 0); \
-        }                                                                                                                           \
-    }
-    BN_STAGE_TAP(0);
-    BN_STAGE_TAP(1);
-    BN_STAGE_TAP(2);
-    {
-        f32x4 acc[2][4];
-#pragma unroll
-        for (int j = 0; j < 2; ++j)
-#pragma unroll
-            for (int T = 0; T < 4; ++T) acc[j][T] = f32x4{0.f, 0.f, 0.f, 0.f};
-#pragma unroll
-        for (int tap = 0; tap < 9; ++tap) {
-            if (tap <= 6) asm volatile("s_waitcnt vmcnt(4) lgkmcnt(0)\n\ts_barrier" ::: "memory");
-            else if (tap == 7) asm volatile("s_waitcnt vmcnt(2) lgkmcnt(0)\n\ts_barrier" ::: "memory");
-            else asm volatile("s_waitcnt vmcnt(0) lgkmcnt(0)\n\ts_barrier" ::: "memory");
-            if (tap + 3 < 9) BN_STAGE_TAP(tap + 3);
-            const int ky = tap / 3, kx = tap - ky * 3;
-            const unsigned char* wb = lds + BN_WBUF + (tap & 3) * 8192;
-            frag_t wf[4][2];
-#pragma unroll
-            for (int T = 0; T < 4; ++T)
-#pragma unroll
-                for (int k = 0; k < 2; ++k) wf[T][k] = *reinterpret_cast<const frag_t*>(wb + BN_SW(T * 16 + l15, k * 4 + g));
+                for (int T = 0; T < 4; ++T) acc[i][T] = f32x4{0.f, 0.f, 0.f, 0.f};
+#pragma unroll
+            for (int k = 0; k < NK32; ++k) {
+                frag_t wf[4];
+#pragma unroll
+                for (int T = 0; T < 4; ++T) {
+                    const int rho = T * 16 + l15;
+                    wf[T] = *reinterpret_cast<const frag_t*>(lds + BN_W1 + (k >> 1) * 8192 + BN_SW(rho, (k & 1) * 4 + g));
+                }
+#pragma unroll
+                for (int i = 0; i < 3; ++i)
+#pragma unroll
+                    for (int T = 0; T < 4; ++T) acc[i][T] = BnFrag<TI>::mfma(wf[T], xf[i][k], acc[i][T]);
+            }
+            const float* s_b1 = reinterpret_cast<const float*>(lds + BN_BIAS);
+#pragma unroll
+            for (int i = 0; i < 3; ++i) {
+                const int hr = wid * 48 + i * 16 + l15;
+#pragma unroll
+                for (int p = 0; p < 2; ++p) {
+                    const float4 ba = *reinterpret_cast<const float4*>(s_b1 + 32 * p + 8 * g), bb = *reinterpret_cast<const float4*>(s_b1 + 32 * p + 8 * g + 4);
+                    const float bias[8] = {ba.x, ba.y, ba.z, ba.w, bb.x, bb.y, bb.z, bb.w};
+                    frag_t o;
+#pragma unroll
+                    for (int e = 0; e < 8; ++e) {
+                        const float v = (e < 4 ? acc[i][2 * p][e] : acc[i][2 * p + 1][e - 4]) + bias[e];
+                        o[e] = (TI)(hvalid[i] ? fmaxf(v, 0.f) : 0.f);
+                    }
+                    *reinterpret_cast<frag_t*>(mid + BN_SW(hr, 4 * p + g)) = o;
+                }
+            }
+        }
+        BN_BARRIER();
+        BN_STAMP(1);
+        nxt = bn_tile(a, 2 * (pair + pair_step) + half);
+        if (pair + pair_step >= pair_end) nxt.ok = false;
+        BN_HALO_ADDR(nxt);
+
+        {
+            int lx = l15;
+            asm volatile("" : "+v"(lx));
+            f32x4 acc[2][4];
+#pragma unroll
+            for (int j = 0; j < 2; ++j)
+#pragma unroll
+                for (int T = 0; T < 4; ++T) acc[j][T] = f32x4{0.f, 0.f, 0.f, 0.f};
+#pragma unroll
+            for (int tap = 0; tap < 9; ++tap) {
+#pragma unroll
+                for (int q = 0; q < 3 * NK32; ++q)
+                    if (q * 9 / (3 * NK32) == tap) BN_HALO_LOAD(q / NK32, q % NK32);
+                __builtin_amdgcn_sched_barrier(0);
+                const int ky = tap / 3, kx = tap - ky * 3;
+                const unsigned char* wb = lds + BN_W2 + tap * 8192;
+                frag_t wf[4][2];
+#pragma unroll
+                for (int T = 0; T < 4; ++T)
+#pragma unroll
+                    for (int k = 0; k < 2; ++k) wf[T][k] = *reinterpret_cast<const frag_t*>(wb + BN_SW(T * 16 + l15, k * 4 + g));
+#pragma unroll
+                for (int j = 0; j < 2; ++j) {
+                    const int hr = (wid * 2 + j + ky) * BN_HW + kx + lx;
+#pragma unroll
+                    for (int k = 0; k < 2; ++k) {
+                        const frag_t af = *reinterpret_cast<const frag_t*>(mid + BN_SW(hr, k * 4 + g));
+#pragma unroll
+                        for (int T = 0; T < 4; ++T) acc[j][T] = BnFrag<TI>::mfma(wf[T][k], af, acc[j][T]);
+                    }
+                }
+            }
+            BN_BARRIER();
+            const float* s_b2 = reinterpret_cast<const float*>(lds + BN_BIAS) + 64;
 #pragma unroll
             for (int j = 0; j < 2; ++j) {
-                const int hr = (wid * 2 + j + ky) * BN_HW + kx + l15;
-#pragma unroll
-                for (int k = 0; k < 2; ++k) {
-                    const frag_t af = *reinterpret_cast<const frag_t*>(lds + BN_MID1 + BN_SW(hr, k * 4 + g));
-#pragma unroll
-                    for (int T = 0; T < 4; ++T) acc[j][T] = BnFrag<TI>::mfma(wf[T][k], af, acc[j][T]);
-                }
-            }
-        }
-        const float* s_b2 = reinterpret_cast<const float*>(lds + BN_BIAS) + 64;
-#pragma unroll
-        for (int j = 0; j < 2; ++j) {
-            const int row = (wid * 2 + j) * 16 + l15;
-#pragma unroll
-            for (int p = 0; p < 2; ++p) {
-                const float4 ba = *reinterpret_cast<const float4*>(s_b2 + 32 * p + 8 * g), bb = *reinterpret_cast<const float4*>(s_b2 + 32 * p + 8 * g + 4);
-                const float bias[8] = {ba.x, ba.y, ba.z, ba.w, bb.x, bb.y, bb.z, bb.w};
-                frag_t o;
-#pragma unroll
-                for (int e = 0; e < 8; ++e) o[e] = (TI)fmaxf((e < 4 ? acc[j][2 * p][e] : acc[j][2 * p + 1][e - 4]) + bias[e], 0.f);
-                *reinterpret_cast<frag_t*>(lds + BN_MID2 + BN_SW(row, 4 * p + g)) = o;
-            }
-        }
-    }
-    __syncthreads();
-    BN_STAMP(3);
-
-    const float* s_b3 = reinterpret_cast<const float*>(lds + BN_BIAS) + 128 + wid * 64;
-    float bias3[2][8];
-#pragma unroll
-    for (int p = 0; p < 2; ++p) {
-        const float4 ba = *reinterpret_cast<const float4*>(s_b3 + 32 * p + 8 * g), bb = *reinterpret_cast<const float4*>(s_b3 + 32 * p + 8 * g + 4);
-        bias3[p][0] = ba.x; bias3[p][1] = ba.y; bias3[p][2] = ba.z; bias3[p][3] = ba.w;
-        bias3[p][4] = bb.x; bias3[p][5] = bb.y; bias3[p][6] = bb.z; bias3[p][7] = bb.w;
-    }
-    frag_t aux[2][2][2];
-    unsigned ooff[2][2];
+                const int row = (wid * 2 + j) * 16 + l15;
+#pragma unroll
+                for (int p = 0; p < 2; ++p) {
+                    const float4 ba = *reinterpret_cast<const float4*>(s_b2 + 32 * p + 8 * g), bb = *reinterpret_cast<const float4*>(s_b2 + 32 * p + 8 * g + 4);
+                    const float bias[8] = {ba.x, ba.y, ba.z, ba.w, bb.x, bb.y, bb.z, bb.w};
+                    frag_t o;
+#pragma unroll
+                    for (int e = 0; e < 8; ++e) o[e] = (TI)fmaxf((e < 4 ? acc[j][2 * p][e] : acc[j][2 * p + 1][e - 4]) + bias[e], 0.f);
+                    *reinterpret_cast<frag_t*>(mid + BN_SW(row, 4 * p + g)) = o;
+                }
+            }
+        }
+        BN_BARRIER();
+        BN_STAMP(2);
+
+        {
+            const float* s_b3 = reinterpret_cast<const float*>(lds + BN_BIAS) + 128 + wid * 64;
+            frag_t aux[2][2][2];
+            unsigned ooff[2][2];
 #define BN_FETCH(buf, gi_)                                                                                                          \
     {                                                                                                                               \
         _Pragma("unroll") for (int j_ = 0; j_ < 2; ++j_) {                                                                          \
-            const int gy_ = y0 + 2 * (gi_) + j_, gx_ = x0 + l15;                                                                    \
-            const bool ok_ = gy_ < a.h && gx_ < a.w;                                                                                \
-            const long long pix_ = ((long long)img * a.h + gy_) * a.w + gx_;                                                        \
+            const int gy_ = cur.y0 + 2 * (gi_) + j_, gx_ = cur.x0 + l15;                                                            \
+            const bool ok_ = cur.ok && gy_ < a.h && gx_ < a.w;                                                                      \
+            const long long pix_ = ((long long)cur.img * a.h + gy_) * a.w + gx_;                                                    \
             ooff[buf][j_] = ok_ ? (unsigned)(pix_ * 256 * 2) : BN_OOB;                                                              \
             _Pragma("unroll") for (int q_ = 0; q_ < 2; ++q_) {                                                                      \
                 const unsigned off_ = !ok_ ? BN_OOB : PROJ ? (unsigned)(pix_ * CIN * 2 + (q_ * 32 + g * 8) * 2)                      \
@@ -269,76 +287,98 @@
             }                                                                                                                       \
         }                                                                                                                           \
     }
-    BN_FETCH(0, 0);
-#pragma unroll
-    for (int gi = 0; gi < 4; ++gi) {
-        const int cur = gi & 1;
-        if (gi + 1 < 4) { BN_FETCH((gi + 1) & 1, gi + 1); }
-        f32x4 acc[2][4];
-#pragma unroll
-        for (int j = 0; j < 2; ++j)
-#pragma unroll
-            for (int T = 0; T < 4; ++T) acc[j][T] = f32x4{0.f, 0.f, 0.f, 0.f};
-#pragma unroll
-        for (int j = 0; j < 2; ++j) {
-            const int row = (2 * gi + j) * 16 + l15;
-#pragma unroll
-            for (int k = 0; k < 2; ++k) {
-                const frag_t af = *reinterpret_cast<const frag_t*>(lds + BN_MID2 + BN_SW(row, k * 4 + g));
-#pragma unroll
-                for (int T = 0; T < 4; ++T) acc[j][T] = BnFrag<TI>::mfma(w3f[T][k], af, acc[j][T]);
-            }
-            if constexpr (PROJ) {
-#pragma unroll
-                for (int k = 0; k < 2; ++k)
-#pragma unroll
-                    for (int T = 0; T < 4; ++T) acc[j][T] = BnFrag<TI>::mfma(wscf[T][k], aux[cur][j][k], acc[j][T]);
-            }
-        }
-#pragma unroll
-        for (int j = 0; j < 2; ++j)
-#pragma unroll
-            for (int p = 0; p < 2; ++p) {
-                frag_t o;
-#pragma unroll
-                for (int e = 0; e < 8; ++e) {
-                    float v = (e < 4 ? acc[j][2 * p][e] : acc[j][2 * p + 1][e - 4]) + bias3[p][e];
-                    if constexpr (!PROJ) v += (float)aux[cur][j][p][e];
-                    o[e] = (TI)fmaxf(v, 0.f);
-                }
-                union { frag_t f; bnu32x4 u; } cv;
-                cv.f = o;
-                __builtin_amdgcn_raw_buffer_store_b128(cv.u, rs_y, ooff[cur][j] == BN_OOB ? BN_OOB : ooff[cur][j] + (unsigned)((wid * 64 + 32 * p + 8 * g) * 2), 0, 0);
-            }
-    }
-    BN_STAMP(4);
+            BN_FETCH(0, 0);
+#pragma unroll
+            for (int gi = 0; gi < 4; ++gi) {
+                const int cb = gi & 1;
+                if (gi + 1 < 4) { BN_FETCH((gi + 1) & 1, gi + 1); }
+                asm volatile("" ::: "memory");
+                float bias3[2][8];
+#pragma unroll
+                for (int p = 0; p < 2; ++p) {
+                    const float4 ba = *reinterpret_cast<const float4*>(s_b3 + 32 * p + 8 * g), bb = *reinterpret_cast<const float4*>(s_b3 + 32 * p + 8 * g + 4);
+                    bias3[p][0] = ba.x; bias3[p][1] = ba.y; bias3[p][2] = ba.z; bias3[p][3] = ba.w;
+                    bias3[p][4] = bb.x; bias3[p][5] = bb.y; bias3[p][6] = bb.z; bias3[p][7] = bb.w;
+                }
+                f32x4 acc[2][4];
+#pragma unroll
+                for (int j = 0; j < 2; ++j)
+#pragma unroll
+                    for (int T = 0; T < 4; ++T) acc[j][T] = f32x4{0.f, 0.f, 0.f, 0.f};
+#pragma unroll
+                for (int j = 0; j < 2; ++j) {
+                    const int row = (2 * gi + j) * 16 + l15;
+#pragma unroll
+                    for (int k = 0; k < 2; ++k) {
+                        const frag_t af = *reinterpret_cast<const frag_t*>(mid + BN_SW(row, k * 4 + g));
+#pragma unroll
+                        for (int T = 0; T < 4; ++T) acc[j][T] = BnFrag<TI>::mfma(w3f[T][k], af, acc[j][T]);
+                    }
+                    if constexpr (PROJ) {
+#pragma unroll
+                        for (int k = 0; k < 2; ++k)
+#pragma unroll
+                            for (int T = 0; T < 4; ++T) acc[j][T] = BnFrag<TI>::mfma(wscf[T][k], aux[cb][j][k], acc[j][T]);
+                    }
+                }
+#pragma unroll
+                for (int j = 0; j < 2; ++j)
+#pragma unroll
+                    for (int p = 0; p < 2; ++p) {
+                        frag_t o;
+#pragma unroll
+                        for (int e = 0; e < 8; ++e) {
+                            float v = (e < 4 ? acc[j][2 * p][e] : acc[j][2 * p + 1][e - 4]) + bias3[p][e];
+                            if constexpr (!PROJ) v += (float)aux[cb][j][p][e];
+                            o[e] = (TI)fmaxf(v, 0.f);
+                        }
+                        union { frag_t f; bnu32x4 u; } cv;
+                        cv.f = o;
+                        __builtin_amdgcn_raw_buffer_store_b128(cv.u, rs_y, ooff[cb][j] == BN_OOB ? BN_OOB : ooff[cb][j] + (unsigned)((wid * 64 + 32 * p + 8 * g) * 2), 0, 0);
+                    }
+            }
+        }
+        BN_STAMP(3);
+        BN_BARRIER();
 #ifdef BN_STAMPS
-    asm volatile("s_waitcnt vmcnt(0)" ::: "memory");
-    BN_STAMP(5);
+        asm volatile("s_waitcnt vmcnt(0)" ::: "memory");
+        BN_STAMP(4);
 #endif
+        cur = nxt;
+    }
+}
+
+static int bn_cu_count() {
+    static std::atomic<int> cus[64];
+    int dev = 0;
+    const bool known = hipGetDevice(&dev) == hipSuccess && dev >= 0 && dev < 64;
+    int c = known ? cus[dev].load(std::memory_order_relaxed) : 0;
+    if (c > 0) return c;
+    if (hipDeviceGetAttribute(&c, hipDeviceAttributeMultiprocessorCount, known ? dev : 0) != hipSuccess || c < 1) return 0;
+    if (known) cus[dev].store(c, std::memory_order_relaxed);
+    return c;
 }
 
 template <class TI>
-static osr_status bottleneck_launch(const osr_bottleneck_params* p, BnArgs& a, hipStream_t st) {
-    const unsigned grid = (unsigned)(a.n * a.tiles_y * a.tiles_x);
+static osr_status bottleneck_launch(const osr_bottleneck_params* p, BnArgs& a, unsigned grid, hipStream_t st) {
     if (p->has_proj) {
         static osr_dev_mask m{0};
         osr_once_per_device(m, [] { (void)hipFuncSetAttribute(reinterpret_cast<const void*>(bottleneck64_kernel<TI, 64, 1>), hipFuncAttributeMaxDynamicSharedMemorySize, BN_LDS); });
-        hipLaunchKernelGGL((bottleneck64_kernel<TI, 64, 1>), dim3(grid), dim3(256), BN_LDS, st, a);
+        hipLaunchKernelGGL((bottleneck64_kernel<TI, 64, 1>), dim3(grid), dim3(512), BN_LDS, st, a);
     } else {
         static osr_dev_mask m{0};
         osr_once_per_device(m, [] { (void)hipFuncSetAttribute(reinterpret_cast<const void*>(bottleneck64_kernel<TI, 256, 0>), hipFuncAttributeMaxDynamicSharedMemorySize, BN_LDS); });
-        hipLaunchKernelGGL((bottleneck64_kernel<TI, 256, 0>), dim3(grid), dim3(256), BN_LDS, st, a);
+        hipLaunchKernelGGL((bottleneck64_kernel<TI, 256, 0>), dim3(grid), dim3(512), BN_LDS, st, a);
     }
     OSR_CHECK_LAUNCH("osr_bottleneck_fwd");
     return OSR_OK;
 }
 
-extern "C" osr_status osr_bottleneck_fwd(const osr_bottleneck_params* p, const void* in, const void* w1, const float* b1, const void* w2,
-                                         const float* b2, const void* w3, const float* b3, const void* wsc, const float* bsc, void* out,
-                                         void* stream) {
+extern "C" osr_status osr_bottleneck_fwd_ex(const osr_bottleneck_params* p, const void* in, const void* w1, const float* b1, const void* w2,
+                                            const float* b2, const void* w3, const float* b3, const void* wsc, const float* bsc, void* out,
+                                            int32_t max_workgroups, void* stream) {
     OSR_REQUIRE(p && in && w1 && b1 && w2 && b2 && w3 && b3 && out, OSR_ERR_INVALID_ARG, "osr_bottleneck_fwd: null pointer");
-    OSR_REQUIRE(p->n >= 1 && p->h >= 1 && p->w >= 1, OSR_ERR_INVALID_ARG, "osr_bottleneck_fwd: bad geometry");
+    OSR_REQUIRE(p->n >= 1 && p->h >= 1 && p->w >= 1 && max_workgroups >= 0, OSR_ERR_INVALID_ARG, "osr_bottleneck_fwd: bad geometry");
     OSR_REQUIRE(p->dtype == OSR_F16 || p->dtype == OSR_BF16, OSR_ERR_UNSUPPORTED, "osr_bottleneck_fwd: dtype must be f16/bf16");
     OSR_REQUIRE(p->cmid == 64 && p->cout == 256 && ((p->has_proj && p->cin == 64) || (!p->has_proj && p->cin == 256)), OSR_ERR_UNSUPPORTED,
                 "osr_bottleneck_fwd: only the res2 shapes are fused (cmid 64, cout 256; cin 64 with a projection or cin 256 without): run "
@@ -359,7 +399,19 @@
 #endif
     a.x_bytes = (unsigned)xb; a.y_bytes = (unsigned)yb;
     a.w1_bytes = (unsigned)(64 * p->cin * 2); a.w2_bytes = 64 * 9 * 64 * 2; a.w3_bytes = 256 * 64 * 2; a.wsc_bytes = (unsigned)(256 * p->cin * 2);
-    OSR_REQUIRE((long long)a.n * a.tiles_y * a.tiles_x < (1ll << 31), OSR_ERR_UNSUPPORTED, "osr_bottleneck_fwd: too many tiles");
+    OSR_REQUIRE((long long)a.n * a.tiles_y * a.tiles_x < (1ll << 30), OSR_ERR_UNSUPPORTED, "osr_bottleneck_fwd: too many tiles");
+    a.ntiles = a.n * a.tiles_y * a.tiles_x;
+    a.npairs = (a.ntiles + 1) / 2;
+    int nwg = bn_cu_count();
+    OSR_REQUIRE(nwg >= 1, OSR_ERR_LAUNCH, "osr_bottleneck_fwd: cannot query the device's compute-unit count");
+    if (max_workgroups > 0 && max_workgroups < nwg) nwg = max_workgroups;
+    if (a.npairs < nwg) nwg = a.npairs;
     hipStream_t st = (hipStream_t)stream;
-    return p->dtype == OSR_F16 ? bottleneck_launch<f16_t>(p, a, st) : bottleneck_launch<bf16_t>(p, a, st);
-}
+    return p->dtype == OSR_F16 ? bottleneck_launch<f16_t>(p, a, (unsigned)nwg, st) : bottleneck_launch<bf16_t>(p, a, (unsigned)nwg, st);
+}
+
+extern "C" osr_status osr_bottleneck_fwd(const osr_bottleneck_params* p, const void* in, const void* w1, const float* b1, const void* w2,
+                                         const float* b2, const void* w3, const float* b3, const void* wsc, const float* bsc, void* out,
+                                         void* stream) {
+    return osr_bottleneck_fwd_ex(p, in, w1, b1, w2, b2, w3, b3, wsc, bsc, out, 0, stream);
+}
diff --git a/openset-rcnn_amd/host/_lib.py b/openset-rcnn_amd/host/_lib.py
--- a/openset-rcnn_amd/host/_lib.py
+++ b/openset-rcnn_amd/host/_lib.py
@@ -116,6 +116,7 @@
     "osr_conv2d_chain_fwd": (I32, [C.POINTER(ConvParams), P, P, P, P, P, I32, P, P, P]),
     "osr_conv2d_chain_fwd_ex": (I32, [C.POINTER(ConvParams), P, P, P, P, P, I32, P, P, P, P]),
     "osr_bottleneck_fwd": (I32, [C.POINTER(BottleneckParams), P, P, P, P, P, P, P, P, P, P, P]),
+    "osr_bottleneck_fwd_ex": (I32, [C.POINTER(BottleneckParams), P, P, P, P, P, P, P, P, P, P, I32, P]),
     "osr_resize_tmp_bytes": (I64, [I32, I32]),
     "osr_resize_bilinear_u8": (I32, [P, I32, I32, I64, P, P, I32, P, P, I32, I32, I32, I32, I32, P, I64, P, P]),
     "osr_resize_bilinear_u8_planar": (I32, [P, I32, I32, I32, P, P, I32, P, P, I32, I32, I32, I32, I32, I32, P, I64, P, P]),
diff --git a/openset-rcnn_amd/host/ops.py b/openset-rcnn_amd/host/ops.py
--- a/openset-rcnn_amd/host/ops.py
+++ b/openset-rcnn_amd/host/ops.py
@@ -419,7 +419,7 @@
     return (out, mid) if keep_mid else out
 
 
-def bottleneck(x: torch.Tensor, w1, b1, w2, b2, w3, b3, wsc=None, bsc=None) -> Optional[torch.Tensor]:
+def bottleneck(x: torch.Tensor, w1, b1, w2, b2, w3, b3, wsc=None, bsc=None, max_workgroups: int = 0) -> Optional[torch.Tensor]:
     lib = _lib.load()
     _need(x, name="x")
     if x.dtype not in (torch.float16, torch.bfloat16):
@@ -440,7 +440,8 @@
         if tuple(wsc.shape) != (cout, 1, 1, cin):
             raise OsrError("bottleneck: projection weight shape")
     out = torch.empty((n, h, w, cout), dtype=x.dtype, device=x.device)
-    st = lib.osr_bottleneck_fwd(C.byref(p), _p(x), _p(w1), _p(b1), _p(w2), _p(b2), _p(w3), _p(b3), _p(wsc), _p(bsc), _p(out), _stream())
+    st = lib.osr_bottleneck_fwd_ex(C.byref(p), _p(x), _p(w1), _p(b1), _p(w2), _p(b2), _p(w3), _p(b3), _p(wsc), _p(bsc), _p(out),
+                                   int(max_workgroups), _stream())
     if st == _lib.ERR_UNSUPPORTED:
         return None
     check(st, "osr_bottleneck_fwd")
```
